# Roywangj/AdaptPoint

Hardware: AMD Instinct MI355X
Metric: set-abstraction fwd+bwd point-clouds/sec (B=32,N=1024) (higher is better)
Workload: dtype bf16

## Files before the change

### adaptpoint_amd/_lib.py

```python
import ctypes
import os

_HERE = os.path.dirname(os.path.abspath(__file__))
LIB_PATH = os.path.join(_HERE, "libadaptpoint_amd.so")
if os.environ.get("APN_LIB_PATH"):
    if os.environ.get("APN_ALLOW_UNSAFE_LIB") != "1":
        raise RuntimeError("APN_LIB_PATH is for diagnostic builds: set APN_ALLOW_UNSAFE_LIB=1 with it")
    LIB_PATH = os.path.abspath(os.environ["APN_LIB_PATH"])
REQUIRED_BUILD_FLAGS = ("-ffp-contract=off", "-fno-slp-vectorize")

_c_int, _c_float, _c_void_p = ctypes.c_int, ctypes.c_float, ctypes.c_void_p
_c_double = ctypes.c_double
_c_longlong = ctypes.c_longlong

SIGNATURES = {
    "apn_version": [],
    "apn_furthest_point_sampling": [_c_int] * 3 + [_c_void_p] * 4,
    "apn_ball_query": [_c_int] * 3 + [_c_float, _c_int] + [_c_void_p] * 4,
    "apn_group_points": [_c_int] * 5 + [_c_void_p] * 4,
    "apn_group_points_grad": [_c_int] * 5 + [_c_void_p] * 4,
    "apn_gather_points": [_c_int] * 4 + [_c_void_p] * 4,
    "apn_gather_points_grad": [_c_int] * 4 + [_c_void_p] * 4,
    "apn_resample_points": [_c_int] * 6 + [_c_void_p] * 6,
    "apn_three_nn": [_c_int] * 3 + [_c_void_p] * 5,
    "apn_three_interpolate": [_c_int] * 4 + [_c_void_p] * 5,
    "apn_three_interpolate_grad": [_c_int] * 4 + [_c_void_p] * 5,
    "apn_furthest_point_sampling_tuned": [_c_int] * 3 + [_c_void_p] * 3 + [_c_int] * 2 + [_c_void_p],
    "apn_fps_debug_stamps": [_c_int] * 3 + [_c_void_p] * 5,
    "apn_furthest_point_sampling_xyz": [_c_int] * 3 + [_c_void_p] * 5,
    "apn_ball_query_zero": [_c_int] * 3 + [_c_float, _c_int] + [_c_void_p] * 4,
    "apn_sa_grid_blocks": [_c_int] * 2,
    "apn_sa_grid_rows": [_c_int] * 3,
    "apn_sa_bwd_main_rows": [_c_int] * 2,
    "apn_sa_acc_words": [_c_int],
    "apn_sa_debug_stamps": [_c_void_p],
    "apn_zero_fill": [_c_void_p, _c_longlong, _c_void_p],
    "apn_debug_stamp": [_c_void_p, _c_int, _c_void_p],
    "apn_debug_vgpr_hold": [_c_int, _c_int, _c_void_p, _c_void_p],
    "apn_debug_vpk_probe": [_c_int, _c_int, _c_int, _c_void_p, _c_void_p],
    "apn_sa_geo_dd_doubles": [_c_int],
    "apn_sa_point_geo": [_c_int] * 4 + [_c_float] + [_c_void_p] * 6,
    "apn_sa_prep_rows": [_c_int] * 2,
    "apn_sa_prep_stats": [_c_int] * 2 + [_c_void_p] * 4 + [_c_int] * 2 + [_c_void_p] * 3 + [_c_longlong, _c_void_p],
    "apn_sa_reduce_rows": [_c_void_p, _c_int, _c_int, _c_double, _c_void_p, _c_void_p],
    "apn_sa_reduce_acc": [_c_void_p, _c_int, _c_double, _c_void_p, _c_void_p],
    "apn_sa_bn_fold": [_c_void_p, _c_int, _c_void_p, _c_int, _c_double, _c_void_p, _c_void_p,
                       _c_float, _c_float, _c_void_p, _c_void_p, _c_void_p, _c_int, _c_void_p,
                       _c_void_p, _c_int, _c_void_p, _c_void_p],
    "apn_sa_fwd_main": [_c_int] * 4 + [_c_float] + [_c_void_p] * 12 + [_c_float, _c_float, _c_int, _c_double,
                                                                        _c_void_p, _c_int] + [_c_void_p] * 7,
    "apn_sa_fwd_out": [_c_int] * 3 + [_c_void_p] * 8 + [_c_float, _c_float, _c_int, _c_double] + [_c_void_p] * 2
                      + [_c_int] + [_c_void_p] * 3 + [_c_int] + [_c_void_p] * 2 + [_c_longlong, _c_void_p],
    "apn_sa_bwd_prep_rows": [_c_int] * 2,
    "apn_sa_bwd_prep": [_c_int] * 3 + [_c_void_p] + [_c_longlong] * 3 + [_c_void_p] + [_c_int]
                       + [_c_void_p] * 3 + [_c_int] + [_c_void_p] * 8,
    "apn_sa_bwd_main": [_c_int] * 4 + [_c_float] + [_c_void_p] * 11 + [_c_double, _c_int] + [_c_void_p] * 9,
    "apn_sa_bwd_weight_rows": [_c_int] * 2,
    "apn_sa_bwd_point_grads": [_c_int] * 3 + [_c_void_p] * 7 + [_c_double, _c_int] + [_c_void_p] * 2 + [_c_int]
                              + [_c_void_p] * 4 + [_c_float] + [_c_void_p] * 5,
    "apn_sa_bwd_finalize": [_c_void_p, _c_int, _c_float, _c_void_p, _c_void_p, _c_int, _c_void_p, _c_void_p, _c_int]
                           + [_c_void_p] * 11,
    "apn_sa_forward_seq": ([_c_int] * 5 + [_c_float] + [_c_void_p] * 12
                           + [_c_void_p] * 5 + [_c_float, _c_float, _c_int]
                           + [_c_void_p] * 5 + [_c_float, _c_float, _c_int]
                           + [_c_double, _c_int] + [_c_void_p] * 11 + [_c_longlong, _c_void_p]),
    "apn_sa_backward_seq": ([_c_int] * 5 + [_c_float] + [_c_void_p] * 15 + [_c_int] * 3
                            + [_c_double] + [_c_void_p] + [_c_longlong] * 3 + [_c_void_p]
                            + [_c_longlong]
                            + [_c_void_p] * 26),
    "apn_attention_small_max": [],
    "apn_attention_small_fwd": [_c_int] * 3 + [_c_void_p] * 5,
    "apn_attention_small_bwd": [_c_int] * 3 + [_c_void_p] * 8,
    "apn_attention_prep": [_c_int] * 3 + [_c_void_p] * 4 + [_c_int, _c_void_p],
    "apn_attention_fwd": [_c_int] * 3 + [_c_void_p] * 4,
    "apn_attention_bwd": [_c_int] * 3 + [_c_void_p] * 9,
    "apn_pointset_group_rows": [_c_int] * 3,
    "apn_pointset_group_max": [_c_int] * 5 + [_c_void_p] * 8,
    "apn_pointset_group_max_grad": [_c_int] * 5 + [_c_void_p] * 9,
    "apn_sa_wide_grid": [_c_int] * 2,
    "apn_sa_wide_colsum_chunks": [_c_int] * 2,
    "apn_sa_wide_colsum": [_c_void_p, _c_int, _c_int, _c_void_p, _c_void_p, _c_void_p],
    "apn_sa_wide_tilemap_ints": [_c_int] * 2,
    "apn_sa_wide_tilemap": [_c_int] * 3 + [_c_void_p] * 3,
    "apn_sa_wide_tilemap_many": [_c_int] * 4 + [_c_void_p] * 3,
    "apn_sa_rowmap_many": [_c_int] * 4 + [_c_void_p] * 6,
    "apn_sa_rowmap_ints": [_c_int] * 2,
    "apn_sa_rowmap_places": [_c_int] * 3,
    "apn_sa_wide_stats1": [_c_int] * 4 + [_c_void_p] * 6,
    "apn_sa_wide_fwd_main": [_c_int] * 5 + [_c_void_p] * 11,
    "apn_sa_wide_bwd_main": [_c_int] * 5 + [_c_void_p] * 15,
    "apn_sa_wide_wgrad_fused": [_c_int],
    "apn_sa_wide_image": [_c_void_p, _c_int, _c_int, _c_void_p, _c_int, _c_int, _c_int, _c_void_p, _c_void_p],
    "apn_sa_wide_bwd_prep_rows": [_c_int] * 2,
    "apn_sa_wide_bwd_prep": [_c_int] * 3 + [_c_void_p] + [_c_longlong] * 3 + [_c_void_p] * 7,
    "apn_sa_wide_consts2": [_c_void_p, _c_int, _c_void_p, _c_int, _c_void_p, _c_double, _c_int] + [_c_void_p] * 4,
    "apn_sa_wide_consts1": [_c_void_p, _c_int, _c_void_p, _c_int, _c_void_p, _c_double, _c_int] + [_c_void_p] * 4,
    "apn_sa_wide_point_terms": [_c_int] * 4 + [_c_void_p] * 5 + [_c_int, _c_float] + [_c_void_p] * 7,
    "apn_sa_wide_wgrad_splits": [_c_int] * 3,
    "apn_sa_wide_csr": [_c_int] * 3 + [_c_void_p] * 9,
    "apn_sa_wide_fwd_prep": [_c_int] * 6 + [_c_float] + [_c_void_p] * 13,
    "apn_sa_wide_fwd_prep_rows": [_c_int] * 3,
    "apn_sa_wide_out": [_c_int] * 3 + [_c_void_p] * 2 + [_c_int] + [_c_void_p] * 3 + [_c_int] + [_c_void_p] * 2,
    "apn_sa_wide_bwd_mid": [_c_void_p, _c_int, _c_void_p, _c_int, _c_int, _c_void_p, _c_double, _c_int] + [_c_void_p] * 7,
    "apn_sa_wide_bwd_fin": [_c_void_p, _c_int, _c_void_p, _c_int, _c_int, _c_void_p, _c_double, _c_int] + [_c_void_p] * 8,
    "apn_sa_wide_point_grads_rows": [_c_int] * 2,
    "apn_sa_wide_point_grads_cols": [_c_int] * 3,
    "apn_sa_wide_point_grads": [_c_int] * 5 + [_c_float] + [_c_void_p] * 13 + [_c_int] + [_c_void_p] * 9,
    "apn_sa_wide_colsum_f32": [_c_void_p, _c_int, _c_int, _c_void_p, _c_void_p],
    "apn_sa_wide_wgrad": [_c_int] * 5 + [_c_void_p] * 7 + [_c_int] + [_c_void_p] * 2,
    "apn_pw_conv_tiles": [_c_int] * 2,
    "apn_pw_conv_forward": [_c_int] * 5 + [_c_void_p] * 5,
    "apn_pw_bn_act": [_c_int] * 3 + [_c_void_p] * 2 + [_c_int] + [_c_void_p] * 2 + [_c_float] * 2 + [_c_int] * 2
                     + [_c_void_p] * 6,
    "apn_pw_bn_act_grad_splits": [_c_int] * 2,
    "apn_pw_bn_act_grad": [_c_int] * 3 + [_c_void_p] * 3 + [_c_int] * 2 + [_c_void_p] * 5,
    "apn_pw_conv_grad_input": [_c_int] * 5 + [_c_void_p] * 4,
    "apn_pw_conv_grad_weight_splits": [_c_int] * 4,
    "apn_pw_conv_grad_weight": [_c_int] * 5 + [_c_void_p] * 5,
    "apn_deform_forward": [_c_int] * 3 + [_c_void_p] * 6 + [_c_float] + [_c_void_p] * 4,
    "apn_deform_backward": [_c_int] * 3 + [_c_void_p] * 4 + [_c_float] + [_c_void_p] * 7,
    "apn_pw_contract_splits": [_c_int] * 4,
    "apn_pw_contract": [_c_int] * 4 + [_c_void_p, _c_longlong, _c_int, _c_int] * 2 + [_c_void_p, _c_longlong, _c_int, _c_int,
                                                                                         _c_void_p, _c_int, _c_void_p],
    "apn_pw_contract2_splits": [_c_int] * 9,
    "apn_pw_contract2": [_c_int] * 3 + [_c_void_p] * 16,
    "apn_fp_blend_stats": [_c_int] * 4 + [_c_void_p] * 6 + [_c_int] + [_c_void_p] * 4 + [_c_float, _c_int] + [_c_void_p] * 3,
    "apn_pw_transpose": [_c_int] * 3 + [_c_void_p] * 3,
    "apn_three_nn_weights": [_c_longlong] + [_c_void_p] * 3,
    "apn_anchor_transforms": [_c_int] + [_c_void_p] * 3 + [_c_float] * 3 + [_c_void_p] * 3,
    "apn_anchor_transforms_grad": [_c_int] + [_c_void_p] * 3 + [_c_float] * 3 + [_c_void_p] * 4,
    "apn_pw_conv_max_tiles": [_c_int],
    "apn_pw_conv_max_forward": [_c_int] * 5 + [_c_void_p] * 3 + [_c_int] + [_c_void_p] * 5,
    "apn_pw_conv_max_backward": [_c_int] * 4 + [_c_void_p] * 5 + [_c_int] + [_c_void_p] * 5,
    "apn_spectral_norm_blocks": [_c_int] * 2,
    "apn_spectral_norm": [_c_int] * 2 + [_c_void_p, _c_int, _c_float] + [_c_void_p] * 8,
    "apn_spectral_norm_grad": [_c_int] * 2 + [_c_void_p] * 8,
    "apn_spectral_norm_many": [_c_int] + [_c_void_p] * 3 + [_c_int, _c_float] + [_c_void_p] * 8,
    "apn_spectral_norm_grad_many": [_c_int] + [_c_void_p] * 10,
    "apn_sa_sample_overlap": [_c_int] * 3 + [_c_float, _c_int] + [_c_void_p] * 7,
    "apn_sa_sample_seq": [_c_int] * 3 + [_c_float, _c_int] + [_c_void_p] * 8,
    "apn_furthest_point_sampling_nested": [_c_int] * 3 + [_c_void_p] * 6,
    "apn_sa_sample_seq_nested": [_c_int] * 3 + [_c_float, _c_int] + [_c_void_p] * 9,
    "apn_pointwolf_params": [_c_int] * 2 + [_c_void_p, _c_int] + [_c_float] * 3 + [_c_void_p] * 4,
    "apn_rsmix_select": [_c_int] * 3 + [_c_void_p] * 2 + [_c_double, _c_int, _c_int] + [_c_void_p] * 3,
    "apn_rsmix_mix": [_c_int] * 4 + [_c_void_p] * 8,
    "apn_cloud_transform": [_c_int] * 4 + [_c_void_p] * 2 + [_c_int] * 2 + [_c_void_p] * 8,
    "apn_cls_confusion": [_c_int] * 2 + [_c_void_p, _c_int] + [_c_void_p] * 5,
    "apn_la_pool_rows": [_c_int] * 2,
    "apn_la_pool_fwd": [_c_int] * 4 + [_c_float] + [_c_void_p] * 3 + [_c_int] + [_c_void_p] * 7,
    "apn_la_stats_fold": [_c_void_p, _c_int, _c_int, _c_double, _c_void_p, _c_void_p],
    "apn_la_pool_bwd": [_c_int] * 4 + [_c_float] + [_c_void_p] * 11 + [_c_int] + [_c_void_p] * 4,
    "apn_knn_query": [_c_int] * 5 + [_c_void_p] * 5,
    "apn_knn_dilated": [_c_int] * 7 + [_c_void_p] * 6,
    "apn_ec_pool_rows": [_c_int] * 2,
    "apn_ec_pool_fwd": [_c_int] * 4 + [_c_void_p, _c_int] + [_c_void_p] * 7,
    "apn_ec_out": [_c_int] * 3 + [_c_void_p] * 2 + [_c_float] + [_c_void_p] * 2,
    "apn_ec_bwd_prep_rows": [_c_int] * 2,
    "apn_ec_bwd_prep": [_c_int] * 3 + [_c_void_p] + [_c_longlong] * 3 + [_c_void_p] * 2 + [_c_float] + [_c_void_p] * 3,
    "apn_ec_out_res": [_c_int] * 3 + [_c_void_p] * 2 + [_c_float, _c_void_p] + [_c_longlong] * 3 + [_c_void_p] * 2,
    "apn_ec_bwd_prep_act": [_c_int] * 3 + [_c_void_p] + [_c_longlong] * 3 + [_c_void_p] * 2 + [_c_float] + [_c_void_p] * 3,
    "apn_ec_csr": [_c_int] * 3 + [_c_void_p] * 5,
    "apn_ec_pool_bwd": [_c_int] * 4 + [_c_void_p] * 5 + [_c_int] + [_c_void_p] * 4,
    "apn_chamfer_max_points": [],
    "apn_chamfer_forward": [_c_int] * 3 + [_c_void_p] * 7,
    "apn_chamfer_backward": [_c_int] * 3 + [_c_void_p] * 9,
    "apn_emd_max_points": [],
    "apn_emd_one_launch_max": [],
    "apn_emd_cost_parts": [_c_int],
    "apn_emd_ratios": [_c_int] * 3 + [_c_void_p] * 6,
    "apn_emd_match": [_c_int] * 3 + [_c_void_p] * 6,
    "apn_emd_cost": [_c_int] * 3 + [_c_void_p] * 8,
    "apn_emd_cost_grad": [_c_int] * 3 + [_c_void_p] * 9,
    "apn_po_knn_query": [_c_int] * 4 + [_c_void_p] * 7,
    "apn_po_ball_query": [_c_int] * 3 + [_c_float, _c_int] + [_c_void_p] * 6,
    "apn_po_furthest_sampling": [_c_int] * 2 + [_c_void_p] * 6,
    "apn_po_csr": [_c_int] * 3 + [_c_void_p] * 5,
    "apn_po_grouping_fwd": [_c_int] * 4 + [_c_void_p] * 4,
    "apn_po_grouping_bwd": [_c_int] * 4 + [_c_void_p] * 5,
    "apn_po_interpolation_fwd": [_c_int] * 4 + [_c_void_p] * 5,
    "apn_po_interpolation_bwd": [_c_int] * 4 + [_c_void_p] * 6,
    "apn_po_subtraction_fwd": [_c_int] * 4 + [_c_void_p] * 5,
    "apn_po_subtraction_bwd": [_c_int] * 4 + [_c_void_p] * 6,
    "apn_po_aggregation_fwd": [_c_int] * 5 + [_c_void_p] * 6,
    "apn_po_aggregation_bwd": [_c_int] * 5 + [_c_void_p] * 11,
    "apn_pt_rows": [_c_int] * 3,
    "apn_pt_mid_rows": [_c_int] * 3,
    "apn_pt_rel_stats": [_c_int] * 3 + [_c_void_p, _c_int] + [_c_void_p] * 5,
    "apn_pt_fold": [_c_void_p, _c_int, _c_int, _c_void_p, _c_void_p],
    "apn_pt_colsum_rows": [_c_int],
    "apn_pt_colsum": [_c_int, _c_int, _c_void_p, _c_int, _c_void_p, _c_void_p],
    "apn_pt_mid": [_c_int] * 3 + [_c_void_p, _c_int] + [_c_void_p] * 7,
    "apn_pt_attend": [_c_int] * 3 + [_c_void_p, _c_int] + [_c_void_p] * 8,
    "apn_pt_attend_bwd": [_c_int] * 3 + [_c_void_p, _c_int] + [_c_void_p] * 10,
    "apn_pt_mid_bwd": [_c_int] * 3 + [_c_void_p, _c_int] + [_c_void_p] * 9,
    "apn_pt_rel_bwd": [_c_int] * 3 + [_c_void_p, _c_int] + [_c_void_p] * 12 + [_c_int, _c_void_p, _c_void_p],
    "apn_pt_scatter_bwd": [_c_int] * 3 + [_c_void_p] * 6 + [_c_int, _c_void_p],
    "apn_vg_scratch_ints": [_c_int],
    "apn_vg_voxelize": [_c_int] * 3 + [_c_void_p] + [_c_double] * 3 + [_c_void_p] * 9,
    "apn_vg_mean_fwd": [_c_int] * 3 + [_c_void_p] * 6,
    "apn_vg_mean_bwd": [_c_int] * 3 + [_c_void_p] * 5,
    "apn_rl_moment_rows": [_c_int] * 3,
    "apn_rl_bwd_rows": [_c_int] * 4,
    "apn_rl_moments": [_c_int] * 3 + [_c_void_p] * 3 + [_c_int] + [_c_void_p] * 3,
    "apn_rl_fold": [_c_int, _c_void_p, _c_double] + [_c_void_p] * 4 + [_c_float, _c_float, _c_int] + [_c_void_p] * 6,
    "apn_rl_forward": [_c_int] * 4 + [_c_void_p] * 3 + [_c_int] + [_c_void_p] * 4,
    "apn_rl_backward": [_c_int] * 4 + [_c_void_p] * 3 + [_c_int] + [_c_void_p] * 6,
    "apn_rl_finalize": [_c_int, _c_int, _c_void_p, _c_void_p, _c_double] + [_c_void_p] * 4 + [_c_int] + [_c_void_p] * 3,
    "apn_ag_moment_rows": [_c_int],
    "apn_ag_point_rows": [_c_int],
    "apn_ag_moments": [_c_int] * 5 + [_c_void_p] * 5,
    "apn_ag_fold": [_c_int] * 2 + [_c_void_p] * 3,
    "apn_ag_combine_fwd": [_c_int] * 5 + [_c_void_p] * 7 + [_c_int] + [_c_void_p] * 4 + [_c_float, _c_int] + [_c_void_p] * 3,
    "apn_ag_combine_bwd": [_c_int] * 5 + [_c_void_p] * 11,
    "apn_ag_sigma_bwd": [_c_int] * 5 + [_c_void_p] * 11,
    "apn_ag_res_relu_max": [_c_int] * 4 + [_c_void_p] * 5,
    "apn_ag_res_relu_max_grad": [_c_int] * 4 + [_c_void_p] * 6,
}

_lib = None


class ExtensionMissing(RuntimeError):
    pass


def load():
    global _lib
    if _lib is not None:
        return _lib
    if not os.path.exists(LIB_PATH):
        raise ExtensionMissing(
            f"{LIB_PATH} not found: build it with `python -m adaptpoint_amd.build` "
            "(hipcc --offload-arch=gfx950). There is no fallback path.")
    lib = ctypes.CDLL(LIB_PATH)
    for name, argtypes in SIGNATURES.items():
        fn = getattr(lib, name)
        fn.argtypes = argtypes
        fn.restype = _c_int
    lib.apn_error_string.argtypes = [_c_int]
    lib.apn_error_string.restype = ctypes.c_char_p
    lib.apn_build_flags.argtypes = []
    lib.apn_build_flags.restype = ctypes.c_char_p
    flags = lib.apn_build_flags().decode("utf-8", "replace").split()
    missing = [f for f in REQUIRED_BUILD_FLAGS if f not in flags]
    if missing and os.environ.get("APN_ALLOW_UNSAFE_LIB") != "1":
        raise ExtensionMissing(f"{LIB_PATH} was built without {missing} (its flags: {' '.join(flags)}): rebuild with "
                               "`python -m adaptpoint_amd.build --force`")
    _lib = lib
    return lib


def check(code, what):
    if code != 0:
        msg = load().apn_error_string(code).decode("utf-8", "replace")
        raise RuntimeError(f"{what} failed: {msg} (code {code})")
```

### adaptpoint_amd/csrc/sa_glue.hip

```cpp
#include "apn_common.h"
#include "sa_chain.h"
#include "apn_mfma.h"

namespace apn {

#ifdef APN_WG_STAMPS
__device__ unsigned long long *d_wg_stamps = nullptr;
__device__ __forceinline__ void wg_stamp(int k) {
    unsigned long long *st = d_wg_stamps;
    if (st && threadIdx.x == 0)
        st[((size_t)blockIdx.y * gridDim.x + blockIdx.x) * 16 + k] = wall_clock64();
}
#else
__device__ __forceinline__ void wg_stamp(int) {}
#endif


typedef __attribute__((ext_vector_type(8))) __bf16 bf16x8;

__device__ __forceinline__ void block_sum_rows(const float *__restrict__ part, int rows, int ncol,
                                               const double *__restrict__ sums, double *out) {
    __shared__ double red[1024 * 4];
    const int t = threadIdx.x;
    if (!part) {
        if (t < ncol) out[t] = sums[t];
        __syncthreads();
        return;
    }
    const int quads = ncol >> 2, q = t % quads, g = t / quads, groups = 1024 / quads;
    const float4 *__restrict__ p4 = (const float4 *)part;
    double s0 = 0.0, s1 = 0.0, s2 = 0.0, s3 = 0.0;
    int r = g;
    for (; r + 7 * groups < rows; r += 8 * groups) {
        float4 v[8];
#pragma unroll
        for (int u = 0; u < 8; ++u) v[u] = p4[(size_t)(r + u * groups) * quads + q];
#pragma unroll
        for (int u = 0; u < 8; ++u) {
            s0 += (double)v[u].x; s1 += (double)v[u].y; s2 += (double)v[u].z; s3 += (double)v[u].w;
        }
    }
    for (; r < rows; r += groups) {
        const float4 v = p4[(size_t)r * quads + q];
        s0 += (double)v.x; s1 += (double)v.y; s2 += (double)v.z; s3 += (double)v.w;
    }
    double *mine = red + (size_t)g * ncol + 4 * q;
    mine[0] = s0; mine[1] = s1; mine[2] = s2; mine[3] = s3;
    __syncthreads();
    for (int st = groups >> 1; st > 0; st >>= 1) {
        if (g < st) {
            const double *other = mine + (size_t)st * ncol;
#pragma unroll
            for (int j = 0; j < 4; ++j) mine[j] += other[j];
        }
        __syncthreads();
    }
    if (t < ncol) out[t] = red[t];
    __syncthreads();
}

__global__ __launch_bounds__(1024) void reduce_rows_kernel(const float *__restrict__ part, int rows,
                                                           int ncol, double count,
                                                           double *__restrict__ out) {
    __shared__ double s[128];
    block_sum_rows(part, rows, ncol, nullptr, s);
    if (threadIdx.x < ncol) out[threadIdx.x] = s[threadIdx.x];
    if (threadIdx.x == 0) { out[ncol] = count; out[ncol + 1] = 1.0; }
}

__device__ __forceinline__ void slice_sum_rows(const float *__restrict__ part, int rows, int quads,
                                               int qa, int qb, double (*red)[4]) {
    const int t = threadIdx.x, grp = t >> 1;
    const float4 *__restrict__ p4 = reinterpret_cast<const float4 *>(part) + ((t & 1) ? qb : qa);
    double s0 = 0.0, s1 = 0.0, s2 = 0.0, s3 = 0.0;
    int r = grp;
    for (; r + 3 * 128 < rows; r += 4 * 128) {
        float4 v[4];
#pragma unroll
        for (int u = 0; u < 4; ++u) v[u] = p4[(size_t)(r + 128 * u) * quads];
#pragma unroll
        for (int u = 0; u < 4; ++u) {
            s0 += (double)v[u].x; s1 += (double)v[u].y; s2 += (double)v[u].z; s3 += (double)v[u].w;
        }
    }
    for (; r < rows; r += 128) {
        const float4 v = p4[(size_t)r * quads];
        s0 += (double)v.x; s1 += (double)v.y; s2 += (double)v.z; s3 += (double)v.w;
    }
    red[t][0] = s0; red[t][1] = s1; red[t][2] = s2; red[t][3] = s3;
    __syncthreads();
    for (int st = 64; st > 0; st >>= 1) {
        if (grp < st) {
#pragma unroll
            for (int j = 0; j < 4; ++j) red[t][j] += red[t + 2 * st][j];
        }
        __syncthreads();
    }
}

__global__ __launch_bounds__(256) void bn_fold_kernel(
    const float *__restrict__ part, int rows, const double *__restrict__ sums_in, int c, double count,
    const float *__restrict__ gamma, const float *__restrict__ beta, float eps, float momentum,
    float *__restrict__ running_mean, float *__restrict__ running_var, long long *__restrict__ nbt,
    int training, float *__restrict__ pack, const float *__restrict__ sgn_gamma, int sgn_c,
    float *__restrict__ sgn_out) {
    __shared__ double red[256][4];
    const int t = threadIdx.x, i = blockIdx.x * 4 + t;
    float g32 = 1.0f, b32 = 0.0f, rm = 0.0f, rv = 1.0f;
    if (t < 4) {
        if (gamma) g32 = gamma[i];
        if (beta) b32 = beta[i];
        if (running_mean) { rm = running_mean[i]; rv = running_var[i]; }
    }
    if (blockIdx.x == 0) {
        if (t == 0 && training && nbt) *nbt += 1;
        if (sgn_out)
            for (int k = t; k < sgn_c; k += 256) sgn_out[k] = (!sgn_gamma || sgn_gamma[k] >= 0.0f) ? 1.0f : -1.0f;
    }
    double sum = 0.0, sumsq = 0.0;
    if (training) {
        if (part) {
            slice_sum_rows(part, rows, c / 2, blockIdx.x, c / 4 + blockIdx.x, red);
            if (t < 4) { sum = red[0][t]; sumsq = red[1][t]; }
        } else if (t < 4) {
            sum = sums_in[i];
            sumsq = sums_in[c + i];
            count = sums_in[2 * c];
        }
    }
    if (t >= 4) return;
    double mean, var;
    if (training) {
        mean = sum / count;
        var = sumsq / count - mean * mean;
        if (var < 0.0) var = 0.0;
        if (running_mean) {
            const double unbiased = var * (count / (count > 1.0 ? count - 1.0 : 1.0));
            running_mean[i] = (float)((1.0 - momentum) * rm + momentum * mean);
            running_var[i] = (float)((1.0 - momentum) * rv + momentum * unbiased);
        }
    } else {
        mean = rm;
        var = rv;
    }
    const double inv = 1.0 / sqrt(var + (double)eps);
    const double g = g32, b = b32;
    pack[i] = (float)(g * inv);
    pack[c + i] = (float)(b - mean * g * inv);
    pack[2 * c + i] = (float)mean;
    pack[3 * c + i] = (float)inv;
}

template <int NT, int QT, int WST, int FST>
__device__ __forceinline__ void stage_skip_operands(int cloud, int n, int m, int m0,
                                                    const __bf16 *__restrict__ ft,
                                                    const __bf16 *__restrict__ ft_lo,
                                                    const int *__restrict__ fidx,
                                                    const float *__restrict__ ws,
                                                    float (*sws)[WST], float (*sfi)[FST], int *ssrc) {
    constexpr int G = NT / 32, QPT = QT / G, WPT = 64 / G;
    const int tid = threadIdx.x, i = tid & 31, q0 = tid >> 5;
    int src[QPT];
#pragma unroll
    for (int t = 0; t < QPT; ++t) {
        const int q = m0 + q0 + G * t;
        const int got = fidx[(size_t)cloud * m + (q < m ? q : m - 1)];
        src[t] = q < m ? got : -1;
    }
    float wv[WPT];
#pragma unroll
    for (int t = 0; t < WPT; ++t) wv[t] = ws[(q0 + G * t) * 32 + i];
    const __bf16 *lo_tab = ft_lo ? ft_lo : ft;
    __bf16 hv[QPT], lv[QPT];
#pragma unroll
    for (int t = 0; t < QPT; ++t) {
        const size_t o = ((size_t)cloud * n + (src[t] < 0 ? 0 : src[t])) * 32 + i;
        hv[t] = ft[o];
        lv[t] = lo_tab[o];
    }
    float v[QPT];
#pragma unroll
    for (int t = 0; t < QPT; ++t) {
        const float f = (float)hv[t] + (ft_lo ? (float)lv[t] : 0.0f);
        v[t] = src[t] >= 0 ? f : 0.0f;
    }
#pragma unroll
    for (int t = 0; t < QPT; ++t) {
        sfi[q0 + G * t][i] = v[t];
        if (ssrc && i == 0) ssrc[q0 + G * t] = src[t] < 0 ? 0 : src[t];
    }
#pragma unroll
    for (int t = 0; t < WPT; ++t) sws[q0 + G * t][i] = wv[t];
}

template <int QT>
__global__ __launch_bounds__(QT * 16) void fwd_out_kernel(int n, int m, const float *__restrict__ ysel,
                                                          const unsigned long long *__restrict__ acc2,
                                                          const double *__restrict__ sums2, BnArgs bn2,
                                                          float *__restrict__ pack2,
                                                          const __bf16 *__restrict__ ft,
                                                          const __bf16 *__restrict__ ft_lo,
                                                          const int *__restrict__ fidx,
                                                          const float *__restrict__ ws,
                                                          const float *__restrict__ bs, int relu,
                                                          float *__restrict__ out, float4 *__restrict__ zero,
                                                          long long zero_n4) {
    constexpr int NT = QT * 16, NW = NT / 64, HALVES = 64 / QT;
    __shared__ float tile[QT][65];
    __shared__ __attribute__((aligned(16))) float sfi[QT][36];
    __shared__ double ftot[128];
    __shared__ float s_sc[64], s_sh[64];
    const bool first = blockIdx.x == 0 && blockIdx.y == 0;
    critical_stream_priority();
    wg_stamp(0);
    double count2 = bn2.count;
    double g2pre = 1.0, b2pre = 0.0;
    if (threadIdx.x < 64) {
        if (bn2.gamma) g2pre = (double)bn2.gamma[threadIdx.x];
        if (bn2.beta) b2pre = (double)bn2.beta[threadIdx.x];
    }
    if (bn2.training) {
        if (threadIdx.x < 128) ftot[threadIdx.x] = sums2 ? sums2[threadIdx.x] : acc_read(acc2, 128, threadIdx.x);
        if (sums2) count2 = sums2[128];
    }
    __shared__ __attribute__((aligned(16))) float sws[64][36];
    __shared__ float s_bs[64];
    const int cloud = blockIdx.y, m0 = blockIdx.x * QT;
    const int tx = threadIdx.x & 63, ty = threadIdx.x >> 6;
    if (threadIdx.x >= 128 && threadIdx.x < 192) s_bs[tx] = (ws && bs) ? bs[tx] : 0.0f;
    float ys4[4];
#pragma unroll
    for (int k = 0; k < 4; ++k) {
        const int q = m0 + ty + NW * k;
        ys4[k] = ysel[((size_t)cloud * m + (q < m ? q : m - 1)) * 64 + tx];
    }
    if (ws) stage_skip_operands<NT, QT, 36, 36>(cloud, n, m, m0, ft, ft_lo, fidx, ws, sws, sfi, nullptr);
    wg_stamp(1);
    __syncthreads();
    wg_stamp(2);
    if (threadIdx.x < 64) {
        if (first && threadIdx.x == 0 && bn2.training && bn2.nbt) *bn2.nbt += 1;
        float sc, sh;
        bn_channel(bn2, 64, threadIdx.x, bn2.training ? ftot[threadIdx.x] : 0.0, bn2.training ? ftot[64 + threadIdx.x] : 0.0,
                   count2, first, pack2, sc, sh, g2pre, b2pre);
        s_sc[threadIdx.x] = sc;
        s_sh[threadIdx.x] = sh;
    }
    __syncthreads();
    {
        const float sc = s_sc[tx], sh = s_sh[tx];
#pragma unroll
        for (int k = 0; k < 4; ++k) {
            const int j = ty + NW * k;
            tile[j][tx] = m0 + j < m ? ys4[k] * sc + sh : 0.f;
        }
    }
    wg_stamp(3);
    __syncthreads();
    wg_stamp(4);
    if (ws) {
        constexpr int QB = QT / 32;
        if (ty < 2 * QB) {
            const int cb = ty & 1, qb = ty >> 1, r = tx & 31, h = tx >> 5;
            f32x16 acc = {0};
#pragma unroll
            for (int st = 0; st < 2; ++st) {
                float av[8], bv[8];
                const float4 a0 = *reinterpret_cast<const float4 *>(&sws[32 * cb + r][16 * st + 8 * h]);
                const float4 a1 = *reinterpret_cast<const float4 *>(&sws[32 * cb + r][16 * st + 8 * h + 4]);
                const float4 b0 = *reinterpret_cast<const float4 *>(&sfi[32 * qb + r][16 * st + 8 * h]);
                const float4 b1 = *reinterpret_cast<const float4 *>(&sfi[32 * qb + r][16 * st + 8 * h + 4]);
                av[0] = a0.x; av[1] = a0.y; av[2] = a0.z; av[3] = a0.w; av[4] = a1.x; av[5] = a1.y; av[6] = a1.z; av[7] = a1.w;
                bv[0] = b0.x; bv[1] = b0.y; bv[2] = b0.z; bv[3] = b0.w; bv[4] = b1.x; bv[5] = b1.y; bv[6] = b1.z; bv[7] = b1.w;
                acc = mfma<2>(make_frag<2>(av), make_frag<2>(bv), acc);
            }
            const int ql = 32 * qb + r;
#pragma unroll
            for (int e = 0; e < 16; ++e) {
                const int c = 32 * cb + acc_row(e, h);
                float v = tile[ql][c] + (acc[e] + s_bs[c]);
                if (relu) v = fmaxf(v, 0.0f);
                if (m0 + ql < m) out[((size_t)cloud * 64 + c) * m + m0 + ql] = v;
            }
        }
    } else {
        const int ql = tx % QT, hh = tx / QT;
#pragma unroll
        for (int k = 0; k < 4; ++k) {
            const int c = 4 * (ty * HALVES + hh) + k;
            float v = tile[ql][c];
            if (relu) v = fmaxf(v, 0.0f);
            if (m0 + ql < m) out[((size_t)cloud * 64 + c) * m + m0 + ql] = v;
        }
    }
    wg_stamp(5);
    if (zero) {
        const long long nb = (long long)gridDim.x * gridDim.y, bid = (long long)blockIdx.y * gridDim.x + blockIdx.x;
        for (long long i = bid * NT + threadIdx.x; i < zero_n4; i += nb * NT) zero[i] = make_float4(0.f, 0.f, 0.f, 0.f);
    }
    wg_stamp(6);
}

template <int QT>
__global__ __launch_bounds__(QT * 16) void bwd_prep_kernel(int n, int m, const float *__restrict__ g_out,
                                                           long long gs_b, long long gs_c, long long gs_m,
                                                           const float *__restrict__ out, int relu,
                                                           const float *__restrict__ ysel,
                                                           const float *__restrict__ pack2,
                                                           const __bf16 *__restrict__ ft,
                                                           const __bf16 *__restrict__ ft_lo,
                                                           const int *__restrict__ fidx,
                                                           const float *__restrict__ ws,
                                                           float *__restrict__ goa,
                                                           unsigned long long *__restrict__ accS,
                                                           float *__restrict__ partWs,
                                                           float *__restrict__ gip,
                                                           const int *__restrict__ dup) {
    constexpr int NT = QT * 16, NW = NT / 64, HALVES = 64 / QT;
    __shared__ float tile[QT][65];
    __shared__ float red[NW][2][64];
    __shared__ __attribute__((aligned(16))) float sfi[QT][36];
    __shared__ float sws[64][33];
    __shared__ int ssrc[QT];
    constexpr int DW = QT == 32 ? 4 : 2;
    __shared__ float sdfi[DW][QT][33];
    const int cloud = blockIdx.y, m0 = blockIdx.x * QT;
    const int tx = threadIdx.x & 63, ty = threadIdx.x >> 6;
    const int ql = tx % QT, hh = tx / QT;
    critical_stream_priority();
    wg_stamp(0);
    const bool distinct = dup && dup[cloud] == 0;
    const int qc = m0 + ql < m ? m0 + ql : m - 1;
    const float *outp = relu ? out : g_out;
    float gv[4], ov[4];
#pragma unroll
    for (int k = 0; k < 4; ++k) {
        const int c = (ty + NW * k) * HALVES + hh;
        gv[k] = g_out[cloud * gs_b + c * gs_c + qc * gs_m];
        ov[k] = relu ? outp[((size_t)cloud * 64 + c) * m + qc] : 1.0f;
    }
    float ys[4];
#pragma unroll
    for (int k = 0; k < 4; ++k) {
        const int q = m0 + ty + NW * k;
        ys[k] = ysel[((size_t)cloud * m + (q < m ? q : m - 1)) * 64 + tx];
    }
    if (ws) stage_skip_operands<NT, QT, 33, 36>(cloud, n, m, m0, ft, ft_lo, fidx, ws, sws, sfi, ssrc);
#pragma unroll
    for (int k = 0; k < 4; ++k) {
        const int c = (ty + NW * k) * HALVES + hh;
        tile[ql][c] = (m0 + ql < m && ov[k] > 0.0f) ? gv[k] : 0.0f;
    }
    const float sc = pack2[tx], mu = pack2[128 + tx], iv = pack2[192 + tx];
    wg_stamp(1);
    __syncthreads();
    wg_stamp(2);
    float s1 = 0.0f, s2 = 0.0f;
#pragma unroll
    for (int k = 0; k < 4; ++k) {
        const int j = ty + NW * k, q = m0 + j;
        if (q < m) {
            const float g = tile[j][tx];
            const float gs = g * sc;
            goa[((size_t)cloud * m + q) * 64 + tx] = gs;
            s1 += g;
            s2 += g * ((ys[k] - mu) * iv);
        }
    }
    red[ty][0][tx] = s1;
    red[ty][1][tx] = s2;
    wg_stamp(3);
    __syncthreads();
    wg_stamp(4);
    const size_t blk = (size_t)blockIdx.y * gridDim.x + blockIdx.x;
    float sacc = 0.0f;
    if (ty < 2) {
#pragma unroll
        for (int k = 0; k < NW; ++k) sacc += red[k][ty][tx];
    }
    wg_stamp(5);
    if (ws) {
        constexpr int QB = QT / 32;
        const int r = tx & 31, h = tx >> 5;
        if (ty < DW * QB) {
            const int qb = ty / DW, part = ty % DW;
            f32x16 acc = {0};
#pragma unroll
            for (int s4 = 0; s4 < 4 / DW; ++s4) {
                const int st = (4 / DW) * part + s4;
                float av[8], bv[8];
#pragma unroll
                for (int j = 0; j < 8; ++j) {
                    av[j] = tile[32 * qb + r][16 * st + 8 * h + j];
                    bv[j] = sws[16 * st + 8 * h + j][r];
                }
                acc = mfma<2>(make_frag<2>(av), make_frag<2>(bv), acc);
            }
#pragma unroll
            for (int e = 0; e < 16; ++e)
                sdfi[part][32 * qb + acc_row(e, h)][r] = acc[e];
        } else if (ty < DW * QB + 2) {
            const int cb = ty - DW * QB;
            f32x16 acc = {0};
#pragma unroll
            for (int st = 0; st < QT / 16; ++st) {
                float av[8], bv[8];
#pragma unroll
                for (int j = 0; j < 8; ++j) {
                    av[j] = tile[16 * st + 8 * h + j][32 * cb + r];
                    bv[j] = sfi[16 * st + 8 * h + j][r];
                }
                acc = mfma<2>(make_frag<2>(av), make_frag<2>(bv), acc);
            }
#pragma unroll
            for (int e = 0; e < 16; ++e)
                partWs[blk * 2048 + (32 * cb + acc_row(e, h)) * 32 + r] = acc[e];
        }
        __syncthreads();
#pragma unroll
        for (int k = 0; k < QT * 32 / NT; ++k) {
            const int o = threadIdx.x + NT * k, q = o >> 5, i = o & 31;
            float v = sdfi[0][q][i] + sdfi[1][q][i];
            if (DW == 4) v += sdfi[DW - 2][q][i] + sdfi[DW - 1][q][i];
            float *dst = gip + ((size_t)cloud * n + ssrc[q]) * 32 + i;
            if (m0 + q < m) {
                if (distinct) *dst = v;
                else atomicAdd(dst, v);
            }
        }
        wg_stamp(6);
    }
    if (ty < 2) acc_add(accS, 128, (int)(blk % ACC_COPIES), ty * 64 + tx, sacc);
    wg_stamp(7);
}

constexpr int WG_PTS = 64;
constexpr int PG_NT = 512, PG_K = WG_PTS * 32 / PG_NT, PG_M = 32 * 64 / PG_NT;
constexpr int PG_RB = 8;

__global__ __launch_bounds__(PG_NT) void bwd_point_grads_kernel(
    int n, int total_q, int split, const float *__restrict__ GU, const int *__restrict__ pcnt,
    const int *__restrict__ poff, const long long *__restrict__ geo,
    const float *__restrict__ HA, const float *__restrict__ HB, const unsigned long long *__restrict__ accT,
    const double *__restrict__ sumsT, double count, int train1,
    const float *__restrict__ pack1, const __bf16 *__restrict__ ft,
    const __bf16 *__restrict__ ft_lo, const float *__restrict__ xyz,
    const float *__restrict__ new_xyz, const float *__restrict__ w1, const float *__restrict__ gip,
    float inv_r, float *__restrict__ partW, float *__restrict__ g_f, float *__restrict__ g_p,
    float *__restrict__ g_q) {
    __shared__ __attribute__((aligned(16))) float swt[35][36];
    __shared__ __attribute__((aligned(16))) float swr[32][36];
    __shared__ float sG[WG_PTS][33];
    __shared__ float sH[WG_PTS][33];
    __shared__ float sI[WG_PTS][33];
    __shared__ float sB[WG_PTS][41];
    __shared__ float sGeo[WG_PTS][4];
    __shared__ float sc[5][32];
    const int tid = threadIdx.x;
    critical_stream_priority();
    wg_stamp(0);
    const int cloud = blockIdx.y, n0 = blockIdx.x * WG_PTS;
    const int block = cloud * gridDim.x + blockIdx.x;
    const size_t p0 = (size_t)cloud * n + n0;
    const int q0 = block * WG_PTS;
    const int n_here = n - n0 < WG_PTS ? n - n0 : WG_PTS;
    const int c_ld = tid & 31;
    float f_hi[PG_K], f_lo[PG_K], g_i[PG_K], h_a[PG_K], h_b[PG_K];
    const int g_pt = tid >> 3, g_c4 = (tid & 7) * 4;
    int r_cnt, r_off;
    {
        const size_t gp = p0 + (g_pt < n_here ? g_pt : 0);
        r_cnt = g_pt < n_here ? pcnt[gp] : 0;
        r_off = poff[gp];
    }
    float4 a_g = make_float4(0.f, 0.f, 0.f, 0.f);
    {
        const __bf16 *lo_tab = ft_lo ? ft_lo : ft;
        const float *gip_tab = gip ? gip : HA;
#pragma unroll
        for (int k = 0; k < PG_K; ++k) {
            const int pt = (tid >> 5) + (PG_NT / 32) * k;
            const size_t pr = (p0 + (pt < n_here ? pt : 0)) * 32 + c_ld;
            const size_t qr = (size_t)(q0 + pt < total_q ? q0 + pt : 0) * 32 + c_ld;
            f_hi[k] = (float)ft[pr];
            f_lo[k] = (float)lo_tab[pr];
            g_i[k] = gip_tab[gip ? pr : qr];
            h_a[k] = HA[qr];
            h_b[k] = HB[qr];
        }
    }
    float xq_v[2] = {0.0f, 0.0f};
    long long geo_v = 0ll;
    if (tid < WG_PTS * 3) {
        const int pt = tid / 3, d = tid % 3;
        xq_v[0] = xyz[(p0 + (pt < n_here ? pt : 0)) * 3 + d];
        xq_v[1] = new_xyz[(size_t)(q0 + pt < total_q ? q0 + pt : 0) * 3 + d];
    } else if (tid >= PG_NT - WG_PTS * 4) {
        const int e = tid - (PG_NT - WG_PTS * 4), pt = e >> 2, j = e & 3;
        geo_v = geo[(p0 + (pt < n_here ? pt : 0)) * 4 + j];
    }
    for (int e = tid; e < 32 * 35; e += PG_NT) {
        const int mid = e / 35, col = e % 35;
        const float w = w1[e];
        const __bf16 hi = (__bf16)w;
        float wr = (float)hi;
        if (split) wr += (float)(__bf16)(w - wr);
        swt[col][mid] = w;
        swr[mid][col < 3 ? 32 + col : col - 3] = wr;
    }
    if (tid < 64) {
        const int c = tid & 31;
        const float sca = pack1[c];
        float val = 0.0f;
        if (train1) {
            const double t = sumsT ? sumsT[tid] : acc_read(accT, 64, tid);
            const double cnt = sumsT ? sumsT[64] : count;
            val = (float)(-(double)sca * t / cnt);
        }
        sc[tid < 32 ? 2 : 1][c] = val;
        if (tid < 32) sc[0][c] = sca;
    } else if (tid >= 96 && tid < 160) sc[3 + ((tid - 96) >> 5)][tid & 31] = pack1[64 + tid - 96];
    {
        const float *rows = GU + (size_t)(r_cnt > 0 ? r_off : 0) * 32 + g_c4;
        for (int j0 = 0; j0 < r_cnt; j0 += PG_RB) {
            float4 v[PG_RB];
#pragma unroll
            for (int u = 0; u < PG_RB; ++u) {
                const int j = j0 + u < r_cnt ? j0 + u : r_cnt - 1;
                v[u] = *reinterpret_cast<const float4 *>(rows + (size_t)j * 32);
            }
#pragma unroll
            for (int u = 0; u < PG_RB; ++u)
                if (j0 + u < r_cnt) { a_g.x += v[u].x; a_g.y += v[u].y; a_g.z += v[u].z; a_g.w += v[u].w; }
        }
    }
    wg_stamp(1);
    __syncthreads();
    wg_stamp(2);
    {
        const int c = tid & 31;
        const float ca = sc[0][c], cb = sc[1][c], cc = sc[2][c];
#pragma unroll
        for (int k = 0; k < PG_K; ++k) {
            const int pt = (tid >> 5) + (PG_NT / 32) * k;
            const bool ok = pt < n_here;
            sB[pt][6 + c] = ok ? f_hi[k] + (ft_lo ? f_lo[k] : 0.0f) : 0.0f;
            sI[pt][c] = (gip && ok) ? g_i[k] : 0.0f;
            sH[pt][c] = q0 + pt < total_q ? __builtin_fmaf(ca, h_a[k], __builtin_fmaf(cb, h_b[k], cc * 32.0f)) : 0.0f;
        }
    }
    sG[g_pt][g_c4] = a_g.x; sG[g_pt][g_c4 + 1] = a_g.y;
    sG[g_pt][g_c4 + 2] = a_g.z; sG[g_pt][g_c4 + 3] = a_g.w;
    if (tid < WG_PTS * 3) {
        const int pt = tid / 3, d = tid % 3;
        const float xv = xq_v[0], qv = xq_v[1];
        sB[pt][d] = pt < n_here ? xv : 0.0f;
        sB[pt][3 + d] = q0 + pt < total_q ? qv : 0.0f;
        sB[pt][38 + d] = 0.0f;
    } else if (tid >= PG_NT - WG_PTS * 4) {
        const int e = tid - (PG_NT - WG_PTS * 4), pt = e >> 2, j = e & 3;
        const long long gv = pt < n_here ? geo_v : 0ll;
        sGeo[pt][j] = j == 0 ? (float)gv : (float)((double)gv * (1.0 / 68719476736.0));
    }
    wg_stamp(3);
    __syncthreads();
    wg_stamp(4);

    const int tx = tid & 63, ty = tid >> 6;
    {
        const float cnt = sGeo[tx][0], gx = sGeo[tx][1], gy = sGeo[tx][2], gz = sGeo[tx][3];
        float fx[32];
#pragma unroll
        for (int i = 0; i < 32; ++i) fx[i] = sB[tx][6 + i];
#pragma unroll
        for (int mm = 0; mm < PG_M; ++mm) {
            const int mid = PG_M * ty + mm;
            const float4 *wrow = reinterpret_cast<const float4 *>(swr[mid]);
            float accf = 0.0f;
#pragma unroll
            for (int i4 = 0; i4 < 8; ++i4) {
                const float4 w = wrow[i4];
                accf = __builtin_fmaf(w.x, fx[4 * i4], accf);
                accf = __builtin_fmaf(w.y, fx[4 * i4 + 1], accf);
                accf = __builtin_fmaf(w.z, fx[4 * i4 + 2], accf);
                accf = __builtin_fmaf(w.w, fx[4 * i4 + 3], accf);
            }
            const float4 wx = wrow[8];
            const float ys = wx.x * gx + wx.y * gy + wx.z * gz + cnt * accf;
            const float yhs = sc[4][mid] * (ys - cnt * sc[3][mid]);
            sG[tx][mid] = sc[0][mid] * sG[tx][mid] + sc[1][mid] * yhs + sc[2][mid] * cnt;
        }
    }
    wg_stamp(5);
    __syncthreads();
    wg_stamp(6);

    {
        const int r = tx & 31, h = tx >> 5;
        if (ty < 3) {
            const float (*X)[33] = ty == 2 ? sH : sG;
            const int col = ty == 1 ? 32 + r : r;
            const bool mine = ty == 0 ? !(r >= 3 && r <= 5) : (ty == 1 ? r < 6 : (r >= 3 && r <= 5));
            f32x16 acc = {0};
#pragma unroll
            for (int st = 0; st < WG_PTS / 16; ++st) {
                float av[8], bv[8];
#pragma unroll
                for (int j = 0; j < 8; ++j) {
                    av[j] = X[16 * st + 8 * h + j][r];
                    bv[j] = mine ? sB[16 * st + 8 * h + j][col] : 0.0f;
                }
                acc = mfma<2>(make_frag<2>(av), make_frag<2>(bv), acc);
            }
            float *row = partW + (size_t)block * 32 * 38;
            if (mine) {
#pragma unroll
                for (int e = 0; e < 16; ++e) row[acc_row(e, h) * 38 + col] = acc[e];
            }
        } else if (ty < 5) {
            const int pb = ty - 3;
            f32x16 acc = {0};
#pragma unroll
            for (int st = 0; st < 2; ++st) {
                float av[8], bv[8];
                const float4 a0 = *reinterpret_cast<const float4 *>(&swt[3 + r][16 * st + 8 * h]);
                const float4 a1 = *reinterpret_cast<const float4 *>(&swt[3 + r][16 * st + 8 * h + 4]);
                av[0] = a0.x; av[1] = a0.y; av[2] = a0.z; av[3] = a0.w; av[4] = a1.x; av[5] = a1.y; av[6] = a1.z; av[7] = a1.w;
#pragma unroll
                for (int j = 0; j < 8; ++j) bv[j] = sG[32 * pb + r][16 * st + 8 * h + j];
                acc = mfma<2>(make_frag<2>(av), make_frag<2>(bv), acc);
            }
            const int pt = 32 * pb + r;
#pragma unroll
            for (int e = 0; e < 16; ++e) {
                const int i = acc_row(e, h);
                if (pt < n_here) g_f[((size_t)cloud * 32 + i) * n + n0 + pt] = acc[e] + sI[pt][i];
            }
        }
    }
    if (!g_p && !g_q) {
        wg_stamp(7);
        return;
    }

    float gr[32];
#pragma unroll
    for (int mid = 0; mid < 32; ++mid) gr[mid] = sG[tx][mid];
    auto dot_col = [&](const float (&v)[32], int col) {
        const float4 *wcol = reinterpret_cast<const float4 *>(swt[col]);
        float s = 0.0f;
#pragma unroll
        for (int i4 = 0; i4 < 8; ++i4) {
            const float4 w = wcol[i4];
            s = __builtin_fmaf(v[4 * i4], w.x, s);
            s = __builtin_fmaf(v[4 * i4 + 1], w.y, s);
            s = __builtin_fmaf(v[4 * i4 + 2], w.z, s);
            s = __builtin_fmaf(v[4 * i4 + 3], w.w, s);
        }
        return s;
    };
    if (ty < 3 && g_p && tx < n_here) g_p[(p0 + tx) * 3 + ty] += dot_col(gr, ty) * inv_r;
    if (ty >= 4 && ty < 7 && g_q && q0 + tx < total_q) {
        float hr[32];
#pragma unroll
        for (int mid = 0; mid < 32; ++mid) hr[mid] = sH[tx][mid];
        g_q[(size_t)(q0 + tx) * 3 + ty - 4] = -dot_col(hr, ty - 4) * inv_r;
    }
    wg_stamp(7);
}

constexpr int FIN_COLS = 32, FIN_GROUPS = 16;
__device__ __forceinline__ double col_sum(const float *__restrict__ base, int rows, int stride,
                                          int col, int g) {
    double s = 0.0;
    int r = g;
    for (; r + 15 * FIN_GROUPS < rows; r += 16 * FIN_GROUPS) {
        float v[16];
#pragma unroll
        for (int u = 0; u < 16; ++u) v[u] = base[(size_t)(r + FIN_GROUPS * u) * stride + col];
#pragma unroll
        for (int u = 0; u < 16; ++u) s += (double)v[u];
    }
    for (; r + 3 * FIN_GROUPS < rows; r += 4 * FIN_GROUPS) {
        float v[4];
#pragma unroll
        for (int u = 0; u < 4; ++u) v[u] = base[(size_t)(r + FIN_GROUPS * u) * stride + col];
#pragma unroll
        for (int u = 0; u < 4; ++u) s += (double)v[u];
    }
    for (; r < rows; r += FIN_GROUPS) s += (double)base[(size_t)r * stride + col];
    return s;
}

constexpr int FIN_W1 = 32 * 35, FIN_WS = 2048, FIN_W2 = 2048, FIN_SMALL = 64 * 3 + 32 * 2;
constexpr int FIN_TOTAL = FIN_W1 + FIN_WS + FIN_W2 + FIN_SMALL;

__global__ __launch_bounds__(FIN_COLS * FIN_GROUPS) void bwd_finalize_kernel(
    const float *__restrict__ partW, int rowsW, double inv_r, float *__restrict__ g_w1,
    const float *__restrict__ partWs, int rowsS, float *__restrict__ g_ws,
    const float *__restrict__ partW2, int rows2, float *__restrict__ g_w2,
    const unsigned long long *__restrict__ accS, const double *__restrict__ sumsS,
    const unsigned long long *__restrict__ accT, const double *__restrict__ sumsT,
    float *__restrict__ g_bs, float *__restrict__ g_g2, float *__restrict__ g_b2, float *__restrict__ g_g1,
    float *__restrict__ g_b1) {
    __shared__ double red[FIN_GROUPS][FIN_COLS];
    critical_stream_priority();
    const int o = threadIdx.x % FIN_COLS, g = threadIdx.x / FIN_COLS;
    const int e = blockIdx.x * FIN_COLS + o;
    double v = 0.0;
    float *dst = nullptr;
    if (e < FIN_W1) {
        const int mid = e / 35, col = e % 35;
        dst = g_w1 + e;
        if (col < 3)
            v = (col_sum(partW, rowsW, 1216, mid * 38 + col, g) -
                 col_sum(partW, rowsW, 1216, mid * 38 + 3 + col, g)) * inv_r;
        else
            v = col_sum(partW, rowsW, 1216, mid * 38 + 3 + col, g);
    } else if (e < FIN_W1 + FIN_WS) {
        if (g_ws) { dst = g_ws + (e - FIN_W1); v = col_sum(partWs, rowsS, 2048, e - FIN_W1, g); }
    } else if (e < FIN_W1 + FIN_WS + FIN_W2) {
        if (g_w2) { dst = g_w2 + (e - FIN_W1 - FIN_WS); v = col_sum(partW2, rows2, 2048, e - FIN_W1 - FIN_WS, g); }
    } else if (e < FIN_TOTAL) {
        if (g == 0) {
            const int k = e - FIN_W1 - FIN_WS - FIN_W2;
            if (k < 192) {
                const int c = k & 63, which = k >> 6;
                const double scale = (sumsS && which) ? 1.0 / sumsS[129] : 1.0;
                if (which == 0) {
                    if (g_bs) { dst = g_bs + c; v = acc_read(accS, 128, c); }
                } else {
                    const int col = which == 1 ? c : 64 + c;
                    dst = which == 1 ? (g_b2 ? g_b2 + c : nullptr) : (g_g2 ? g_g2 + c : nullptr);
                    if (dst) v = (sumsS ? sumsS[col] : acc_read(accS, 128, col)) * scale;
                }
            } else {
                const int c = (k - 192) & 31, which = (k - 192) >> 5;
                const double scale = sumsT ? 1.0 / sumsT[65] : 1.0;
                dst = which == 0 ? (g_b1 ? g_b1 + c : nullptr) : (g_g1 ? g_g1 + c : nullptr);
                if (dst) v = (sumsT ? sumsT[32 * which + c] : acc_read(accT, 64, 32 * which + c)) * scale;
            }
        }
    }
    red[g][o] = v;
    __syncthreads();
    if (g == 0 && dst) {
        double acc = 0.0;
#pragma unroll
        for (int k = 0; k < FIN_GROUPS; ++k) acc += red[k][o];
        *dst = (float)acc;
    }
}

__global__ __launch_bounds__(128) void reduce_acc_kernel(const unsigned long long *__restrict__ acc, int ncol,
                                                         double count, double *__restrict__ out) {
    const int t = threadIdx.x;
    if (t < ncol) out[t] = acc_read(acc, ncol, t);
    if (t == 0) { out[ncol] = count; out[ncol + 1] = 1.0; }
}

}

#define APN_ST ((hipStream_t)stream)

extern "C" int apn_sa_reduce_rows(const float *part, int rows, int ncol, double count, double *out,
                                  void *stream) {
    if (rows < 0 || ncol < 4 || ncol > 128 || (1024 % ncol) || !part || !out) return APN_EINVAL;
    if ((uintptr_t)part & 15) return APN_EINVAL;
    hipLaunchKernelGGL(apn::reduce_rows_kernel, dim3(1), dim3(1024), 0, APN_ST, part, rows, ncol, count,
                       out);
    APN_LAUNCH_CHECK();
    return APN_OK;
}

extern "C" int apn_sa_reduce_acc(const void *acc, int ncol, double count, double *out, void *stream) {
    if (ncol < 1 || ncol > 128 || !acc || !out) return APN_EINVAL;
    hipLaunchKernelGGL(apn::reduce_acc_kernel, dim3(1), dim3(128), 0, APN_ST, (const unsigned long long *)acc, ncol,
                       count, out);
    APN_LAUNCH_CHECK();
    return APN_OK;
}

extern "C" int apn_sa_bn_fold(const float *part, int rows, const double *sums, int c, double count,
                              const float *gamma, const float *beta, float eps, float momentum,
                              float *running_mean, float *running_var, void *num_batches_tracked,
                              int training, float *pack, const float *sgn_gamma, int sgn_c,
                              float *sgn_out, void *stream) {
    if (c < 4 || c > 1024 || (c & 3) || !pack || sgn_c > 1024) return APN_EINVAL;
    if (training && !part && !sums) return APN_EINVAL;
    if (!training && (!running_mean || !running_var)) return APN_EINVAL;
    if (part && ((uintptr_t)part & 15)) return APN_EINVAL;
    hipLaunchKernelGGL(apn::bn_fold_kernel, dim3(c / 4), dim3(256), 0, APN_ST, part, rows, sums, c, count,
                       gamma, beta, eps, momentum, running_mean, running_var,
                       (long long *)num_batches_tracked, training, pack, sgn_gamma, sgn_c, sgn_out);
    APN_LAUNCH_CHECK();
    return APN_OK;
}

static int apn_sa_glue_tile(int b, int m) { return (long long)b * ((m + 63) / 64) <= 512 ? 32 : 64; }

extern "C" int apn_sa_fwd_out(int b, int n, int m, const float *ysel, const void *acc2, const double *sums2,
                              const float *g2, const float *b2, float *rm2, float *rv2, void *nbt2, float eps2,
                              float mom2, int train2, double count, float *pack2, const void *ft, int precision,
                              const int *fidx, const float *ws, const float *bs, int relu, float *out,
                              float *zero_base, long long zero_floats, void *stream) {
    if (b <= 0 || m <= 0 || b > 65535 || !ysel || !pack2 || !out) return APN_EINVAL;
    if (train2 && !acc2 && !sums2) return APN_EINVAL;
    if (!train2 && (!rm2 || !rv2)) return APN_EINVAL;
    if (ws && (!ft || !fidx || n <= 0 || (precision != 1 && precision != 2))) return APN_EINVAL;
    const __bf16 *hi = (const __bf16 *)ft;
    const __bf16 *lo = (ws && precision == 2) ? hi + (size_t)b * n * 32 : nullptr;
    if (zero_base && (zero_floats < 0 || (zero_floats & 3) || ((uintptr_t)zero_base & 15))) return APN_EINVAL;
    apn::BnArgs bn{g2, b2, rm2, rv2, (long long *)nbt2, eps2, mom2, train2, count};
    if (apn_sa_glue_tile(b, m) == 32)
        hipLaunchKernelGGL(apn::fwd_out_kernel<32>, dim3((m + 31) / 32, b), dim3(512), 0, APN_ST, n, m, ysel,
                           (const unsigned long long *)(sums2 ? nullptr : acc2), sums2, bn, pack2, hi, lo, fidx, ws, bs,
                           relu, out, (float4 *)zero_base, zero_base ? zero_floats / 4 : 0);
    else
        hipLaunchKernelGGL(apn::fwd_out_kernel<64>, dim3((m + 63) / 64, b), dim3(1024), 0, APN_ST, n, m, ysel,
                           (const unsigned long long *)(sums2 ? nullptr : acc2), sums2, bn, pack2, hi, lo, fidx, ws, bs,
                           relu, out, (float4 *)zero_base, zero_base ? zero_floats / 4 : 0);
    APN_LAUNCH_CHECK();
    return APN_OK;
}

extern "C" int apn_sa_bwd_prep_rows(int b, int m) {
    const int qt = apn_sa_glue_tile(b, m);
    return b * ((m + qt - 1) / qt);
}

extern "C" int apn_sa_bwd_prep(int b, int n, int m, const float *g_out, long long gs_b,
                               long long gs_c, long long gs_m, const float *out, int relu,
                               const float *ysel, const float *pack2, const void *ft, int precision,
                               const int *fidx, const float *ws, float *goa, void *accS,
                               float *partWs, float *gip, const int *dup, void *stream) {
    if (b <= 0 || m <= 0 || b > 65535 || !g_out || !ysel || !pack2 || !goa || !accS) return APN_EINVAL;
    if (relu && !out) return APN_EINVAL;
    if (ws && (!ft || !fidx || !partWs || !gip || n <= 0 || (precision != 1 && precision != 2)))
        return APN_EINVAL;
    const __bf16 *hi = (const __bf16 *)ft;
    const __bf16 *lo = (ws && precision == 2) ? hi + (size_t)b * n * 32 : nullptr;
    if (apn_sa_glue_tile(b, m) == 32)
        hipLaunchKernelGGL(apn::bwd_prep_kernel<32>, dim3((m + 31) / 32, b), dim3(512), 0, APN_ST, n, m, g_out,
                           gs_b, gs_c, gs_m, out, relu, ysel, pack2, hi, lo, fidx, ws, goa, (unsigned long long *)accS,
                           partWs, gip, dup);
    else
        hipLaunchKernelGGL(apn::bwd_prep_kernel<64>, dim3((m + 63) / 64, b), dim3(1024), 0, APN_ST, n, m, g_out,
                           gs_b, gs_c, gs_m, out, relu, ysel, pack2, hi, lo, fidx, ws, goa, (unsigned long long *)accS,
                           partWs, gip, dup);
    APN_LAUNCH_CHECK();
    return APN_OK;
}

#ifdef APN_WG_STAMPS
extern "C" __attribute__((visibility("default"))) int apn_sa_debug_wg_stamps(void *buf) {
    return (int)hipMemcpyToSymbol(HIP_SYMBOL(apn::d_wg_stamps), &buf, sizeof(buf));
}
#endif

extern "C" int apn_sa_bwd_weight_rows(int b, int n) { return b * ((n + apn::WG_PTS - 1) / apn::WG_PTS); }

extern "C" int apn_sa_bwd_point_grads(int b, int n, int m, const float *GU, const int *pcnt_poff, const void *geo,
                                      const float *HA, const float *HB, const void *accT, const double *sumsT,
                                      double count, int train1, const float *pack1, const void *ft, int precision,
                                      const float *xyz, const float *new_xyz, const float *w1,
                                      const float *gip, float radius, float *partW, float *g_f,
                                      float *g_p, float *g_newp, void *stream) {
    if (b <= 0 || n <= 0 || m <= 0 || b > 65535) return APN_EINVAL;
    if (!GU || !pcnt_poff || !geo || !HA || !HB || (!accT && !sumsT) || !pack1 || !ft || !xyz || !new_xyz || !w1 || !partW ||
        !g_f)
        return APN_EINVAL;
    if (precision != 1 && precision != 2) return APN_EINVAL;
    if (m > n) return APN_EINVAL;
    const __bf16 *hi = (const __bf16 *)ft;
    const __bf16 *lo = precision == 2 ? hi + (size_t)b * n * 32 : nullptr;
    hipLaunchKernelGGL(apn::bwd_point_grads_kernel, dim3((n + apn::WG_PTS - 1) / apn::WG_PTS, b),
                       dim3(apn::PG_NT), 0, APN_ST, n, b * m, precision == 2 ? 1 : 0, GU, pcnt_poff,
                       pcnt_poff + (size_t)b * n, (const long long *)geo, HA, HB,
                       (const unsigned long long *)accT, sumsT, count, train1,
                       pack1, hi, lo, xyz, new_xyz, w1, gip, 1.0f / radius, partW, g_f, g_p, g_newp);
    APN_LAUNCH_CHECK();
    return APN_OK;
}

extern "C" int apn_sa_bwd_finalize(const float *partW, int rows_w, float radius, float *g_w1,
                                   const float *partWs, int rows_s, float *g_ws, const float *partW2, int rows_2,
                                   float *g_w2, const void *accS, const double *sumsS,
                                   const void *accT, const double *sumsT, float *g_bs, float *g_g2, float *g_b2,
                                   float *g_g1, float *g_b1, void *stream) {
    if (!partW || !g_w1 || (g_ws && !partWs) || (g_w2 && !partW2) || !accS || (!accT && !sumsT))
        return APN_EINVAL;
    hipLaunchKernelGGL(apn::bwd_finalize_kernel, dim3((apn::FIN_TOTAL + apn::FIN_COLS - 1) / apn::FIN_COLS),
                       dim3(apn::FIN_COLS * apn::FIN_GROUPS), 0, APN_ST, partW,
                       rows_w, 1.0 / (double)radius, g_w1, partWs, rows_s, g_ws, partW2, rows_2, g_w2,
                       (const unsigned long long *)accS, sumsS, (const unsigned long long *)accT, sumsT, g_bs,
                       g_g2, g_b2, g_g1, g_b1);
    APN_LAUNCH_CHECK();
    return APN_OK;
}
```

### adaptpoint_amd/csrc/sa_seq.hip

```cpp
#include "apn_common.h"

#define APN_TRY(expr)            \
    do {                         \
        int rc__ = (expr);       \
        if (rc__) return rc__;   \
    } while (0)

namespace apn {
__global__ __launch_bounds__(256) void zero16_kernel(uint4 *__restrict__ p, long long n16) {
    const long long stride = (long long)gridDim.x * 256;
    for (long long e = (long long)blockIdx.x * 256 + threadIdx.x; e < n16; e += stride) p[e] = make_uint4(0, 0, 0, 0);
}
__global__ __launch_bounds__(256) void fill32_kernel(unsigned *__restrict__ p, unsigned word, long long n) {
    const long long stride = (long long)gridDim.x * 256;
    for (long long e = (long long)blockIdx.x * 256 + threadIdx.x; e < n; e += stride) p[e] = word;
}
}

extern "C" int apn_zero_fill(void *base, long long bytes, void *stream) {
    if (bytes < 0 || (bytes & 15) || (bytes && (!base || ((uintptr_t)base & 15)))) return APN_EINVAL;
    if (!bytes) return APN_OK;
    long long blocks = (bytes / 16 + 255) / 256;
    if (blocks > 1024) blocks = 1024;
    hipLaunchKernelGGL(apn::zero16_kernel, dim3((unsigned)blocks), dim3(256), 0, (hipStream_t)stream, (uint4 *)base,
                       bytes / 16);
    APN_LAUNCH_CHECK();
    return APN_OK;
}

extern "C" int apn_sa_forward_seq(
    int phases, int precision, int b, int n, int m, float radius, const float *xyz, const float *new_xyz,
    const float *f, const int *idx, const int *tmap, const int *fidx, const void *geo, const void *dd,
    const float *w1, const float *w2, const float *ws, const float *bs,
    const float *g1, const float *b1, float *rm1, float *rv1, void *nbt1, float eps1, float mom1,
    int train1,
    const float *g2, const float *b2, float *rm2, float *rv2, void *nbt2, float eps2, float mom2,
    int train2,
    double count, int relu, void *ft, float *part1, const double *sums1, const double *sums2,
    float *pack1, float *pack2, void *acc2, float *ysel, void *ksel,
    float *out, float *zero_base, long long zero_floats, void *stream) {
    if (phases & 1)
        APN_TRY(apn_sa_prep_stats(b, n, f, geo, dd, w1, precision, train1, ft, part1, acc2, apn_sa_acc_words(128),
                                  stream));
    if (phases & 2)
        APN_TRY(apn_sa_fwd_main(b, n, m, precision, radius, xyz, new_xyz, ft, idx, tmap, w1, w2, g1, b1, rm1, rv1,
                                nbt1, eps1, mom1, train1, count, part1, apn_sa_prep_rows(b, n), sums1, pack1, g2,
                                ysel, ksel, acc2, stream));
    if (phases & 4)
        APN_TRY(apn_sa_fwd_out(b, n, m, ysel, acc2, sums2, g2, b2, rm2, rv2, nbt2, eps2, mom2, train2, count, pack2,
                               ws ? ft : nullptr, precision, ws ? fidx : nullptr, ws, bs, relu, out, zero_base,
                               zero_floats, stream));
    return APN_OK;
}

extern "C" int apn_sa_backward_seq(
    int phases, int precision, int b, int n, int m, float radius, const float *xyz, const float *new_xyz,
    const int *idx, const int *tmap, const int *fidx, const void *geo, const float *w1, const float *w2,
    const float *ws, const void *ft, const float *pack1, const float *pack2, const float *ysel,
    const void *ksel, const float *out, int relu, int train1, int train2, double count,
    const float *g_out, long long gs_b, long long gs_c, long long gs_m,
    void *zero_base, long long zero_bytes, float *gip, void *accS, void *accT,
    const int *pcnt_poff, const int *rowdst, float *GU,
    float *goa, float *partWs, float *partW2, float *partW, const double *sumsS, const double *sumsT,
    float *HA, float *HB,
    float *g_f, float *g_p, float *g_newp, float *g_w1, float *g_w2, float *g_g1, float *g_b1, float *g_g2,
    float *g_b2, float *g_ws, float *g_bs, void *stream) {
    if (phases & 1) {
        if (zero_bytes) APN_TRY(apn_zero_fill(zero_base, zero_bytes, stream));
        APN_TRY(apn_sa_bwd_prep(b, n, m, g_out, gs_b, gs_c, gs_m, out, relu, ysel, pack2, ws ? ft : nullptr, precision,
                                ws ? fidx : nullptr, ws, goa, accS, partWs, gip,
                                pcnt_poff ? pcnt_poff + 2ll * b * n : nullptr, stream));
    }
    if (phases & 2)
        APN_TRY(apn_sa_bwd_main(b, n, m, precision, radius, xyz, new_xyz, ft, idx, tmap, w1, w2, pack1, pack2, accS,
                                sumsS, count, train2, goa, ksel, accT, partW2, rowdst, GU, HA, HB, stream));
    if (phases & 4) {
        APN_TRY(apn_sa_bwd_point_grads(b, n, m, GU, pcnt_poff, geo, HA, HB, accT, sumsT, count, train1, pack1, ft, precision, xyz,
                                       new_xyz, w1, gip, radius, partW, g_f, g_p, g_newp, stream));
        APN_TRY(apn_sa_bwd_finalize(partW, apn_sa_bwd_weight_rows(b, n), radius, g_w1, partWs,
                                    apn_sa_bwd_prep_rows(b, m), g_ws, partW2, apn_sa_bwd_main_rows(b, m), g_w2, accS,
                                    sumsS, accT, sumsT, g_bs, g_g2, g_b2, g_g1, g_b1, stream));
    }
    return APN_OK;
}

extern "C" int apn_sa_sample_seq_nested(int b, int n, int m, float radius, int nsample, const float *xyz,
                                        const int *tie_prev, int *tie_out, int *fidx, float *new_xyz, int *idx, void *geo,
                                        void *dd, void *stream) {
    if (b <= 0 || n <= 0 || m <= 0 || !tie_out) return APN_EINVAL;
    APN_TRY(apn_furthest_point_sampling_nested(b, n, m, xyz, tie_prev, fidx, new_xyz, tie_out, stream));
    APN_TRY(apn_ball_query_zero(b, n, m, radius, nsample, new_xyz, xyz, idx, stream));
    if (geo) APN_TRY(apn_sa_point_geo(b, n, m, nsample, radius, xyz, new_xyz, idx, geo, dd, stream));
    return APN_OK;
}

extern "C" int apn_sa_sample_seq(int b, int n, int m, float radius, int nsample, const float *xyz,
                                 float *temp, int *fidx, float *new_xyz, int *idx, void *geo, void *dd,
                                 void *stream) {
    if (b <= 0 || n <= 0 || m <= 0) return APN_EINVAL;
    if (temp) {
        long long blocks = ((long long)b * n + 255) / 256;
        if (blocks > 2048) blocks = 2048;
        hipLaunchKernelGGL(apn::fill32_kernel, dim3((unsigned)blocks), dim3(256), 0, (hipStream_t)stream, (unsigned *)temp,
                           0x501502F9u, (long long)b * n);
        APN_LAUNCH_CHECK();
    }
    APN_TRY(apn_furthest_point_sampling_xyz(b, n, m, xyz, temp, fidx, new_xyz, stream));
    APN_TRY(apn_ball_query_zero(b, n, m, radius, nsample, new_xyz, xyz, idx, stream));
    if (geo) APN_TRY(apn_sa_point_geo(b, n, m, nsample, radius, xyz, new_xyz, idx, geo, dd, stream));
    return APN_OK;
}
```

### adaptpoint_amd/fused.py

```python
import torch
import torch.distributed as dist
import torch.nn as nn

from . import _lib
from . import ops as _ops

C_IN, C_MID, C_OUT, K_NS = 32, 32, 64, 32
DETERMINISTIC = True

PRECISION = "bf16x3"
_PREC = {"bf16": 1, "bf16x3": 2}

PER_KERNEL_LAUNCH = False


def covers(B, N, M, K, C, w1, w2, biased=False, momenta=()):
    return (C == C_IN and K == K_NS and tuple(w1) == (C_MID, C_IN + 3) and tuple(w2) == (C_OUT, C_MID) and not biased
            and (M is None or M <= N) and B <= 65535 and all(m is not None for m in momenta))


def supported(p, f, idx_or_k, conv1, conv2, bns=(), npoint=None):
    k = idx_or_k.shape[2] if torch.is_tensor(idx_or_k) else int(idx_or_k)
    m = idx_or_k.shape[1] if torch.is_tensor(idx_or_k) else npoint
    return (f.is_cuda and f.dtype == torch.float32 and p.dtype == torch.float32
            and covers(p.shape[0], p.shape[1], m, k, f.shape[1], conv1.weight.shape[:2], conv2.weight.shape[:2],
                       conv1.bias is not None or conv2.bias is not None, [bn.momentum for bn in bns]))


_FN = {}


def _call(name, dev, *args, stream=None):
    fn = _FN.get(name)
    if fn is None:
        fn = _FN[name] = getattr(_lib.load(), name)
    if stream is None:
        if dev.index is not None and dev.index != torch.cuda.current_device():
            with torch.cuda.device(dev):
                code = fn(*args, torch.cuda.current_stream(dev).cuda_stream)
            if code:
                _lib.check(code, name)
            return
        stream = torch.cuda.current_stream(dev).cuda_stream
    code = fn(*args, stream)
    if code:
        _lib.check(code, name)


class _Launcher:

    def __init__(self, dev):
        self.dev = dev
        if dev.index is not None and dev.index != torch.cuda.current_device():
            self.stream = None
        else:
            self.stream = torch.cuda.current_stream(dev).cuda_stream

    def __call__(self, name, *args):
        _call(name, self.dev, *args, stream=self.stream)


def _ptr(t):
    return None if t is None else t.data_ptr()


FORCE_PHASED = False


def _world(sync):
    if sync and dist.is_available() and dist.is_initialized():
        return dist.get_world_size()
    return 1


def _allreduce_sum_(t):
    if dist.is_available() and dist.is_initialized() and (dist.get_world_size() > 1 or FORCE_PHASED):
        from . import dp
        dp.all_reduce_sum_(t)


def _phased(sync):
    return _world(sync) > 1 or (FORCE_PHASED and sync)


def _carve(dev, sizes, zero=False):
    offs, total = [], 0
    for _, nfl in sizes:
        offs.append(total)
        total += (int(nfl) + 63) // 64 * 64
    buf = (torch.zeros if zero else torch.empty)(max(total, 64), dtype=torch.float32, device=dev)
    return {name: buf[o:o + int(nfl)] for (name, nfl), o in zip(sizes, offs)}, buf


def _all_reduce_rows(call, part, rows, ncol, count, dev):
    sums = torch.empty(ncol + 2, dtype=torch.float64, device=dev)
    call("apn_sa_reduce_rows", part.data_ptr(), rows, ncol, float(count), sums.data_ptr())
    _allreduce_sum_(sums)
    return sums


def _all_reduce_acc(call, acc, ncol, count, dev):
    sums = torch.empty(ncol + 2, dtype=torch.float64, device=dev)
    call("apn_sa_reduce_acc", acc.data_ptr(), ncol, float(count), sums.data_ptr())
    _allreduce_sum_(sums)
    return sums


def _bn_args(bn):
    training = bn.training or not bn.track_running_stats
    track = bn.track_running_stats
    if bn.momentum is None:
        raise RuntimeError("fused set abstraction: BatchNorm(momentum=None) is not covered "
                           "(fused.supported() routes it to the unfused path)")
    mom = bn.momentum
    return (_ptr(bn.weight), _ptr(bn.bias), _ptr(bn.running_mean) if track else None,
            _ptr(bn.running_var) if track else None,
            _ptr(bn.num_batches_tracked) if (track and bn.training) else None,
            float(bn.eps), float(mom), 1 if training else 0)


def _mat(w, rows, cols):
    w = w.detach().reshape(rows, cols)
    return w if w.is_contiguous() else w.contiguous()


def _acc_floats(ncol):
    return 2 * _lib.load().apn_sa_acc_words(ncol)


class _Forward:

    def __init__(self, p, f, new_p, idx, fidx, radius, conv1, bn1, conv2, bn2, skip_conv, relu,
                 sync_bn, tmap=None, geo=None, dd=None, want_backward=False, rowmap=None):
        dev = f.device
        call = _Launcher(dev)
        lib = _lib.load()
        B, C, N = f.shape
        M = new_p.shape[1]
        self.dims = (B, N, M)
        self.radius = float(radius)
        self.sync = sync_bn
        self.relu = 1 if relu else 0
        self.prec = prec = _PREC[PRECISION]
        w1 = _mat(conv1.weight, C_MID, C_IN + 3)
        w2 = _mat(conv2.weight, C_OUT, C_MID)
        ws = bs = None
        if skip_conv is not None:
            ws = _mat(skip_conv.weight, C_OUT, C_IN)
            bs = skip_conv.bias.detach() if skip_conv.bias is not None else None
        count = float(B * M * K_NS)
        if geo is None:
            geo, dd = point_geo(p, new_p, idx, radius)
        if want_backward:
            from . import fused_wide
            if tmap is None:
                tmap = fused_wide.tile_map(idx)
                rowmap = None
            if rowmap is None:
                rowmap = fused_wide.row_map(tmap, B, N, M, fidx=fidx)
        rows1 = lib.apn_sa_prep_rows(B, N)
        v, _buf = _carve(dev, [("ft", prec * B * N * C // 2), ("pack1", 4 * C_MID), ("pack2", 4 * C_OUT),
                               ("ysel", B * M * C_OUT), ("ksel", B * M * C_OUT // 4),
                               ("part1", rows1 * 64), ("acc2", _acc_floats(128))])
        out = torch.empty(B, C_OUT, M, dtype=torch.float32, device=dev)
        self.zsizes = (([("gip", B * N * C_MID)] if ws is not None else [])
                       + [("accS", _acc_floats(128)), ("accT", _acc_floats(64))])
        self.zviews = self.zbuf = None
        if want_backward:
            self.zviews, self.zbuf = _carve(dev, self.zsizes)
        zptr, zfl = _ptr(self.zbuf), (self.zbuf.numel() if self.zbuf is not None else 0)
        bn1a, bn2a = _bn_args(bn1), _bn_args(bn2)
        self.train1, self.train2 = bool(bn1a[7]), bool(bn2a[7])

        def run(phases, sums1=None, sums2=None):
            if PER_KERNEL_LAUNCH:
                return _forward_per_kernel(call, phases, prec, B, N, M, self.radius, p, new_p, f, idx, fidx, geo, dd,
                                           w1, w2, ws, bs, bn1a, bn2a, count, self.relu, v, sums1,
                                           sums2, out, rows1, tmap, zptr, zfl)
            call("apn_sa_forward_seq", phases, prec, B, N, M, self.radius, p.data_ptr(), new_p.data_ptr(),
                 f.data_ptr(), idx.data_ptr(), _ptr(tmap), _ptr(fidx), geo.data_ptr(), dd.data_ptr(),
                 w1.data_ptr(), w2.data_ptr(), _ptr(ws), _ptr(bs), *bn1a, *bn2a, count, self.relu,
                 v["ft"].data_ptr(), v["part1"].data_ptr(), _ptr(sums1), _ptr(sums2),
                 v["pack1"].data_ptr(), v["pack2"].data_ptr(), v["acc2"].data_ptr(),
                 v["ysel"].data_ptr(), v["ksel"].data_ptr(), out.data_ptr(), zptr, zfl)

        if not _phased(sync_bn):
            run(7)
        else:
            run(1)
            s1 = _all_reduce_rows(call, v["part1"], rows1, 64, count, dev) if self.train1 else None
            run(2, sums1=s1)
            s2 = _all_reduce_acc(call, v["acc2"], 128, count, dev) if self.train2 else None
            run(4, sums2=s2)
        self.out = out
        self.saved = dict(p=p, f=f, new_p=new_p, idx=idx, tmap=tmap, rowmap=rowmap, fidx=fidx,
                          geo=geo, ft=v["ft"], w1=w1, w2=w2, ws=ws,
                          has_bs=bs is not None, pack1=v["pack1"], pack2=v["pack2"], ysel=v["ysel"],
                          ksel=v["ksel"], count=count)


def _backward(fw, g_out, need_p, need_newp):
    if fw is None:
        raise RuntimeError("fused set abstraction: backward called a second time (its saved state is "
                           "released after the first backward; retain_graph is not supported)")
    sv = fw.saved
    B, N, M = fw.dims
    dev = fw.out.device
    P, sync = sv["count"], fw.sync
    f32 = dict(dtype=torch.float32, device=dev)
    if g_out is None:
        g_out = torch.zeros_like(fw.out)
    if g_out.dtype != torch.float32:
        g_out = g_out.float()
    gs = g_out.stride()
    w1, w2, ws = sv["w1"], sv["w2"], sv["ws"]
    has_skip = ws is not None
    lib = _lib.load()
    call = _Launcher(dev)
    rows = lib.apn_sa_bwd_main_rows(B, M)
    prow = lib.apn_sa_bwd_prep_rows(B, M)
    wrows = lib.apn_sa_bwd_weight_rows(B, N)

    prezeroed = fw.zbuf is not None
    zsizes = [] if prezeroed else fw.zsizes
    if sv["rowmap"] is None:
        raise RuntimeError("fused set abstraction: backward without a row map (the forward was run with want_backward=False)")
    pcnt_poff, rowdst = sv["rowmap"]
    sizes = zsizes + [("goa", B * M * C_OUT), ("partWs", prow * C_OUT * C_IN if has_skip else 0),
                      ("partW2", rows * C_OUT * C_MID), ("partW", wrows * 32 * 38),
                      ("HA", B * M * C_MID), ("HB", B * M * C_MID), ("GU", lib.apn_sa_rowmap_places(B, N, M) * C_MID)]
    v, buf = _carve(dev, sizes)
    zero_floats = sum((nfl + 63) // 64 * 64 for _, nfl in zsizes)
    if prezeroed:
        v.update(fw.zviews)
        fw.zbuf = fw.zviews = None
    gsz = [("w2", C_OUT * C_MID), ("w1", C_MID * (C_IN + 3)), ("g1", C_MID), ("b1", C_MID),
           ("g2", C_OUT), ("b2", C_OUT), ("ws", C_OUT * C_IN if has_skip else 0),
           ("bs", C_OUT if (has_skip and sv["has_bs"]) else 0)]
    g, _gbuf = _carve(dev, gsz)
    g_f = torch.empty(B, C_IN, N, **f32)
    g_p = _ops.zeros(B, N, 3, **f32) if need_p else None
    g_newp = torch.empty(B, M, 3, **f32) if need_newp else None
    gws = g["ws"].data_ptr() if has_skip else None
    gbs = g["bs"].data_ptr() if (has_skip and sv["has_bs"]) else None

    def run(phases, sumsS=None, sumsT=None):
        if PER_KERNEL_LAUNCH:
            return _backward_per_kernel(call, phases, fw, sv, g_out, buf, zero_floats, v, g, sumsS,
                                        sumsT, g_f, g_p, g_newp, rows, prow, wrows, has_skip, pcnt_poff, rowdst)
        call("apn_sa_backward_seq", phases, fw.prec, B, N, M, fw.radius, sv["p"].data_ptr(),
             sv["new_p"].data_ptr(), sv["idx"].data_ptr(), _ptr(sv["tmap"]), _ptr(sv["fidx"]), sv["geo"].data_ptr(),
             w1.data_ptr(), w2.data_ptr(), _ptr(ws), sv["ft"].data_ptr(), sv["pack1"].data_ptr(),
             sv["pack2"].data_ptr(), sv["ysel"].data_ptr(), sv["ksel"].data_ptr(),
             fw.out.data_ptr(), fw.relu, 1 if fw.train1 else 0, 1 if fw.train2 else 0, float(P),
             g_out.data_ptr(), gs[0], gs[1], gs[2], buf.data_ptr(), zero_floats * 4,
             v["gip"].data_ptr() if has_skip else None, v["accS"].data_ptr(),
             v["accT"].data_ptr(), pcnt_poff.data_ptr(), rowdst.data_ptr(), v["GU"].data_ptr(), v["goa"].data_ptr(),
             v["partWs"].data_ptr() if has_skip else None, v["partW2"].data_ptr(), v["partW"].data_ptr(),
             _ptr(sumsS), _ptr(sumsT), v["HA"].data_ptr(), v["HB"].data_ptr(),
             g_f.data_ptr(), _ptr(g_p), _ptr(g_newp), g["w1"].data_ptr(), g["w2"].data_ptr(),
             g["g1"].data_ptr(), g["b1"].data_ptr(), g["g2"].data_ptr(), g["b2"].data_ptr(), gws, gbs)

    if not _phased(sync):
        run(7)
    else:
        run(1)
        sS = _all_reduce_acc(call, v["accS"], 128, P, dev)
        run(2, sumsS=sS)
        sT = _all_reduce_acc(call, v["accT"], 64, P, dev)
        run(4, sumsS=sS, sumsT=sT)
    return dict(f=g_f, p=g_p, new_p=g_newp, w1=g["w1"].view(C_MID, C_IN + 3, 1, 1),
                w2=g["w2"].view(C_OUT, C_MID, 1, 1), g1=g["g1"], b1=g["b1"], g2=g["g2"], b2=g["b2"],
                ws=g["ws"].view(C_OUT, C_IN, 1) if has_skip else None,
                bs=g["bs"] if (has_skip and sv["has_bs"]) else None)


def _forward_per_kernel(call, phases, prec, B, N, M, radius, p, new_p, f, idx, fidx, geo, dd, w1, w2, ws, bs,
                        bn1a, bn2a, count, relu, v, sums1, sums2, out, rows1, tmap=None, zptr=None, zfl=0):
    lib = _lib.load()
    if phases & 1:
        call("apn_sa_prep_stats", B, N, f.data_ptr(), geo.data_ptr(), dd.data_ptr(), w1.data_ptr(), prec,
             bn1a[7], v["ft"].data_ptr(), v["part1"].data_ptr(), v["acc2"].data_ptr(), lib.apn_sa_acc_words(128))
    if phases & 2:
        call("apn_sa_fwd_main", B, N, M, prec, radius, p.data_ptr(), new_p.data_ptr(), v["ft"].data_ptr(),
             idx.data_ptr(), _ptr(tmap), w1.data_ptr(), w2.data_ptr(), *bn1a, count, v["part1"].data_ptr(), rows1,
             _ptr(sums1), v["pack1"].data_ptr(), bn2a[0], v["ysel"].data_ptr(), v["ksel"].data_ptr(),
             v["acc2"].data_ptr())
    if phases & 4:
        call("apn_sa_fwd_out", B, N, M, v["ysel"].data_ptr(), v["acc2"].data_ptr(), _ptr(sums2), *bn2a, count,
             v["pack2"].data_ptr(), v["ft"].data_ptr() if ws is not None else None, prec,
             _ptr(fidx) if ws is not None else None, _ptr(ws), _ptr(bs), relu, out.data_ptr(), zptr, zfl)


def _backward_per_kernel(call, phases, fw, sv, g_out, buf, zero_floats, v, g, sumsS, sumsT, g_f, g_p,
                         g_newp, rows, prow, wrows, has_skip, pcnt_poff, rowdst):
    B, N, M = fw.dims
    w1, w2, ws, P = sv["w1"], sv["w2"], sv["ws"], float(sv["count"])
    gip = v["gip"].data_ptr() if has_skip else None
    if phases & 1:
        if zero_floats:
            call("apn_zero_fill", buf.data_ptr(), zero_floats * 4)
        call("apn_sa_bwd_prep", B, N, M, g_out.data_ptr(), *g_out.stride(), fw.out.data_ptr(), fw.relu,
             sv["ysel"].data_ptr(), sv["pack2"].data_ptr(), sv["ft"].data_ptr() if has_skip else None,
             fw.prec, _ptr(sv["fidx"]) if has_skip else None, _ptr(ws), v["goa"].data_ptr(),
             v["accS"].data_ptr(), v["partWs"].data_ptr() if has_skip else None, gip,
             pcnt_poff.data_ptr() + 8 * B * N)
    if phases & 2:
        call("apn_sa_bwd_main", B, N, M, fw.prec, fw.radius, sv["p"].data_ptr(), sv["new_p"].data_ptr(),
             sv["ft"].data_ptr(), sv["idx"].data_ptr(), _ptr(sv["tmap"]), w1.data_ptr(), w2.data_ptr(),
             sv["pack1"].data_ptr(), sv["pack2"].data_ptr(), v["accS"].data_ptr(), _ptr(sumsS), P,
             1 if fw.train2 else 0, v["goa"].data_ptr(), sv["ksel"].data_ptr(), v["accT"].data_ptr(),
             v["partW2"].data_ptr(), rowdst.data_ptr(), v["GU"].data_ptr(), v["HA"].data_ptr(), v["HB"].data_ptr())
    if phases & 4:
        call("apn_sa_bwd_point_grads", B, N, M, v["GU"].data_ptr(), pcnt_poff.data_ptr(), sv["geo"].data_ptr(),
             v["HA"].data_ptr(), v["HB"].data_ptr(), v["accT"].data_ptr(), _ptr(sumsT), P, 1 if fw.train1 else 0,
             sv["pack1"].data_ptr(), sv["ft"].data_ptr(), fw.prec, sv["p"].data_ptr(), sv["new_p"].data_ptr(),
             w1.data_ptr(), gip, fw.radius, v["partW"].data_ptr(), g_f.data_ptr(), _ptr(g_p), _ptr(g_newp))
        call("apn_sa_bwd_finalize", v["partW"].data_ptr(), wrows, fw.radius, g["w1"].data_ptr(),
             v["partWs"].data_ptr() if has_skip else None, prow, g["ws"].data_ptr() if has_skip else None,
             v["partW2"].data_ptr(), rows, g["w2"].data_ptr(), v["accS"].data_ptr(), _ptr(sumsS),
             v["accT"].data_ptr(), _ptr(sumsT), g["bs"].data_ptr() if (has_skip and sv["has_bs"]) else None,
             g["g2"].data_ptr(), g["b2"].data_ptr(), g["g1"].data_ptr(), g["b1"].data_ptr())


class _GroupedMlpMax(torch.autograd.Function):
    @staticmethod
    def forward(ctx, p, new_p, f, idx, w1, g1, b1, w2, g2, b2, mods):
        radius, conv1, bn1, conv2, bn2, sync_bn = mods
        fw = _Forward(p.contiguous(), f.contiguous(), new_p.contiguous(), idx.contiguous(), None,
                      radius, conv1, bn1, conv2, bn2, None, False, sync_bn, want_backward=any(ctx.needs_input_grad))
        ctx.fw = fw
        ctx.save_for_backward(p, new_p, f, idx)
        ctx.set_materialize_grads(False)
        ctx.flags = (p.requires_grad, new_p.requires_grad,
                     g1 is not None, b1 is not None, g2 is not None, b2 is not None)
        return fw.out

    @staticmethod
    def backward(ctx, g_out):
        need_p, need_q, a1, a2, a3, a4 = ctx.flags
        ctx.saved_tensors
        g = _backward(ctx.fw, g_out, need_p, need_q)
        ctx.fw = None
        return (g["p"], g["new_p"], g["f"], None, g["w1"], g["g1"] if a1 else None,
                g["b1"] if a2 else None, g["w2"], g["g2"] if a3 else None,
                g["b2"] if a4 else None, None)


def grouped_mlp_max(p, new_p, f, idx, radius, conv1, bn1, conv2, bn2, sync_bn=False):
    return _GroupedMlpMax.apply(p, new_p, f, idx, conv1.weight, bn1.weight, bn1.bias,
                                conv2.weight, bn2.weight, bn2.bias,
                                (radius, conv1, bn1, conv2, bn2, sync_bn))


class Sampling:

    def __init__(self, B, M, K, device):
        self.shape = (B, M, K)
        self.buf = torch.empty(B * M * (1 + 3 + K), dtype=torch.int32, device=device)
        o = 0
        self.fidx = self.buf[o:o + B * M].view(B, M)
        o += B * M
        self.new_p = self.buf[o:o + B * M * 3].view(torch.float32).view(B, M, 3)
        o += B * M * 3
        self.idx = self.buf[o:o + B * M * K].view(B, M, K)
        self.index = None
        self.tmap = None
        self.rowmap = None
        self.geo = None
        self.dd = None
        self.ready = None
        self.ties = None

    def alloc_geo(self, n_points):
        if self.geo is None or self.geo.shape[1] != n_points:
            B = self.shape[0]
            dev = self.buf.device
            self.geo = torch.empty(B, n_points, 4, dtype=torch.int64, device=dev)
            self.dd = torch.empty(B, _lib.load().apn_sa_geo_dd_doubles(n_points), dtype=torch.float64, device=dev)
        return self.geo, self.dd

    def clouds(self, lo, hi):
        v = object.__new__(Sampling)
        for name, t in vars(self).items():
            setattr(v, name, t[lo:hi] if name in _PER_CLOUD and t is not None else None)
        v.shape = (hi - lo,) + self.shape[1:]
        return v


_PER_CLOUD = ("fidx", "new_p", "idx", "geo", "dd", "ties")


@torch.no_grad()
def point_geo(p, new_p, idx, radius, out=None):
    B, N, _ = p.shape
    M, K = idx.shape[1], idx.shape[2]
    dev = p.device
    if out is None:
        geo = torch.empty(B, N, 4, dtype=torch.int64, device=dev)
        dd = torch.empty(B, _lib.load().apn_sa_geo_dd_doubles(N), dtype=torch.float64, device=dev)
    else:
        geo, dd = out
    _Launcher(dev)("apn_sa_point_geo", B, N, M, K, float(radius), p.contiguous().data_ptr(),
                   new_p.contiguous().data_ptr(), idx.contiguous().data_ptr(), geo.data_ptr(), dd.data_ptr())
    return geo, dd


@torch.no_grad()
def sample_and_query(p, npoint, radius, nsample=K_NS, out=None, geo=False, nested=False, ties=None):
    p = p.contiguous()
    dev = p.device
    B, N, _ = p.shape
    smp = out if out is not None else Sampling(B, npoint, nsample, dev)
    assert smp.shape == (B, npoint, nsample)
    gptr = dptr = None
    if geo and nsample == K_NS and smp.buf is not None:
        g_, d_ = smp.alloc_geo(N)
        gptr, dptr = g_.data_ptr(), d_.data_ptr()
    elif geo and nsample == K_NS and smp.geo is not None:
        gptr, dptr = smp.geo.data_ptr(), smp.dd.data_ptr()
    call = _Launcher(dev)
    if nested and N <= 4096:
        if smp.ties is None:
            smp.ties = torch.empty(B, dtype=torch.int32, device=dev)
        if PER_KERNEL_LAUNCH:
            call("apn_furthest_point_sampling_nested", B, N, npoint, p.data_ptr(), _ptr(ties), smp.fidx.data_ptr(),
                 smp.new_p.data_ptr(), smp.ties.data_ptr())
            call("apn_ball_query_zero", B, N, npoint, float(radius), nsample, smp.new_p.data_ptr(), p.data_ptr(),
                 smp.idx.data_ptr())
            if gptr is not None:
                call("apn_sa_point_geo", B, N, npoint, nsample, float(radius), p.data_ptr(), smp.new_p.data_ptr(),
                     smp.idx.data_ptr(), gptr, dptr)
            return smp
        call("apn_sa_sample_seq_nested", B, N, npoint, float(radius), nsample, p.data_ptr(), _ptr(ties), smp.ties.data_ptr(),
             smp.fidx.data_ptr(), smp.new_p.data_ptr(), smp.idx.data_ptr(), gptr, dptr)
        return smp
    if PER_KERNEL_LAUNCH:
        call("apn_furthest_point_sampling_xyz", B, N, npoint, p.data_ptr(), None,
             smp.fidx.data_ptr(), smp.new_p.data_ptr())
        call("apn_ball_query_zero", B, N, npoint, float(radius), nsample, smp.new_p.data_ptr(),
             p.data_ptr(), smp.idx.data_ptr())
        if gptr is not None:
            call("apn_sa_point_geo", B, N, npoint, nsample, float(radius), p.data_ptr(),
                 smp.new_p.data_ptr(), smp.idx.data_ptr(), gptr, dptr)
        return smp
    call("apn_sa_sample_seq", B, N, npoint, float(radius), nsample, p.data_ptr(), None,
         smp.fidx.data_ptr(), smp.new_p.data_ptr(), smp.idx.data_ptr(), gptr, dptr)
    return smp


@torch.no_grad()
def sample_and_query_many(ps, npoint, radius, nsample=K_NS, outs=None):
    ps = [p.contiguous() for p in ps]
    B, N, _ = ps[0].shape
    dev = ps[0].device
    if outs is None:
        outs = [Sampling(B, npoint, nsample, dev) for _ in ps]
    assert len(outs) == len(ps) and all(o.shape == (B, npoint, nsample) for o in outs)
    call = _Launcher(dev)
    for i in range(len(ps) + 1):
        a = i if i < len(ps) else None
        b = i - 1 if i >= 1 else None
        call("apn_sa_sample_overlap", B, N, npoint, float(radius), nsample,
             ps[a].data_ptr() if a is not None else None,
             outs[a].fidx.data_ptr() if a is not None else None,
             outs[a].new_p.data_ptr() if a is not None else None,
             ps[b].data_ptr() if b is not None else None,
             outs[b].new_p.data_ptr() if b is not None else None,
             outs[b].idx.data_ptr() if b is not None else None)
        if b is not None and outs[b].geo is not None:
            point_geo(ps[b], outs[b].new_p, outs[b].idx, radius, out=(outs[b].geo, outs[b].dd))
    return outs


class _SetAbstraction(torch.autograd.Function):
    @staticmethod
    def forward(ctx, p, f, w1, g1, b1, w2, g2, b2, ws, bs, mods):
        npoint, radius, conv1, bn1, conv2, bn2, skip_conv, relu, sync_bn, sampling = mods
        p = p.contiguous()
        f = f.contiguous()
        smp = sampling if sampling is not None else sample_and_query(p, npoint, radius, geo=True)
        fidx, new_p, idx = smp.fidx, smp.new_p, smp.idx
        if p.requires_grad:
            new_p = new_p.clone()
        fw = _Forward(p, f, new_p, idx, fidx, radius, conv1, bn1, conv2, bn2, skip_conv, relu,
                      sync_bn, tmap=smp.tmap, geo=smp.geo, dd=smp.dd, want_backward=any(ctx.needs_input_grad),
                      rowmap=smp.rowmap)
        ctx.fw = fw
        ctx.save_for_backward(p, f)
        ctx.set_materialize_grads(False)
        ctx.flags = (p.requires_grad, g1 is not None, b1 is not None, g2 is not None,
                     b2 is not None, ws is not None, bs is not None)
        ctx.mark_non_differentiable(new_p) if not p.requires_grad else None
        return new_p, fw.out

    @staticmethod
    def backward(ctx, g_newp_in, g_out):
        need_p, a1, a2, a3, a4, a5, a6 = ctx.flags
        fw = ctx.fw
        ctx.saved_tensors
        g = _backward(fw, g_out, need_p, need_p)
        g_p = g["p"]
        if need_p:
            gq = g["new_p"] if g_newp_in is None else g["new_p"] + g_newp_in
            g_p = g_p.scatter_add(1, fw.saved["fidx"].long().unsqueeze(-1).expand(-1, -1, 3), gq)
        ctx.fw = None
        return (g_p, g["f"], g["w1"], g["g1"] if a1 else None, g["b1"] if a2 else None, g["w2"],
                g["g2"] if a3 else None, g["b2"] if a4 else None, g["ws"] if a5 else None,
                g["bs"] if a6 else None, None)


def fused_set_abstraction(p, f, npoint, radius, conv1, bn1, conv2, bn2, skip_conv=None, relu=True,
                          sync_bn=False, sampling=None):
    assert skip_conv is None or isinstance(skip_conv, nn.Conv1d)
    ws = skip_conv.weight if skip_conv is not None else None
    bs = skip_conv.bias if skip_conv is not None else None
    return _SetAbstraction.apply(p, f, conv1.weight, bn1.weight, bn1.bias, conv2.weight, bn2.weight,
                                 bn2.bias, ws, bs,
                                 (npoint, radius, conv1, bn1, conv2, bn2, skip_conv, relu, sync_bn,
                                  sampling))
```

### include/adaptpoint_amd.h

```cpp
#ifndef ADAPTPOINT_AMD_H
#define ADAPTPOINT_AMD_H

#include <stddef.h>

#ifdef __cplusplus
extern "C" {
#endif

#define APN_OK 0
#define APN_EINVAL (-1)

#if defined(__GNUC__)
#define APN_API __attribute__((visibility("default")))
#else
#define APN_API
#endif

APN_API int apn_version(void);

APN_API const char *apn_error_string(int code);

APN_API const char *apn_build_flags(void);

APN_API int apn_furthest_point_sampling(int b, int n, int m, const float *xyz, float *temp,
                                int *idxs, void *stream);

APN_API int apn_ball_query(int b, int n, int m, float radius, int nsample, const float *new_xyz,
                   const float *xyz, int *idx, void *stream);

APN_API int apn_group_points(int b, int c, int n, int npoints, int nsample, const float *points,
                     const int *idx, float *out, void *stream);

APN_API int apn_group_points_grad(int b, int c, int n, int npoints, int nsample,
                          const float *grad_out, const int *idx, float *grad_points,
                          void *stream);

APN_API int apn_gather_points(int b, int c, int n, int npoints, const float *points,
                      const int *idx, float *out, void *stream);

APN_API int apn_gather_points_grad(int b, int c, int n, int npoints, const float *grad_out,
                           const int *idx, float *grad_points, void *stream);

APN_API int apn_resample_points(int b, int n, int c, int p_all, int s_cnt, int cx,
                                const float *points, const int *fidx, const int *choice,
                                float *pos, float *x, void *stream);

APN_API int apn_three_nn(int b, int n, int m, const float *unknown, const float *known,
                 float *dist2, int *idx, void *stream);

APN_API int apn_three_interpolate(int b, int c, int m, int n, const float *points, const int *idx,
                          const float *weight, float *out, void *stream);

APN_API int apn_three_interpolate_grad(int b, int c, int n, int m, const float *grad_out,
                               const int *idx, const float *weight, float *grad_points,
                               void *stream);


APN_API int apn_furthest_point_sampling_xyz(int b, int n, int m, const float *xyz, float *temp,
                                            int *idxs, float *new_xyz, void *stream);

APN_API int apn_ball_query_zero(int b, int n, int m, float radius, int nsample,
                                const float *new_xyz, const float *xyz, int *idx, void *stream);

APN_API int apn_sa_grid_blocks(int b, int m);
APN_API int apn_sa_grid_rows(int b, int m, int with_tile_map);
APN_API int apn_sa_bwd_main_rows(int b, int m);
APN_API int apn_sa_acc_words(int ncol);
APN_API int apn_zero_fill(void *base, long long bytes, void *stream);
APN_API int apn_debug_stamp(void *stamps, int slot, void *stream);
APN_API int apn_debug_vgpr_hold(int blocks, int turns, unsigned long long *bad, void *stream);
APN_API int apn_debug_vpk_probe(int blocks, int turns, int form, unsigned long long *bad, void *stream);


APN_API int apn_sa_geo_dd_doubles(int n);
APN_API int apn_sa_point_geo(int b, int n, int m, int nsample, float radius, const float *xyz,
                             const float *new_xyz, const int *idx, void *geo, void *dd, void *stream);

APN_API int apn_sa_prep_rows(int b, int n);
APN_API int apn_sa_prep_stats(int b, int n, const float *f, const void *geo, const void *dd, const float *w1,
                              int precision, int stats, void *ft, float *part1, void *zero, long long zero_words,
                              void *stream);

APN_API int apn_sa_reduce_rows(const float *part, int rows, int ncol, double count, double *out,
                               void *stream);
APN_API int apn_sa_reduce_acc(const void *acc, int ncol, double count, double *out, void *stream);

APN_API int apn_sa_bn_fold(const float *part, int rows, const double *sums, int c, double count,
                           const float *gamma, const float *beta, float eps, float momentum,
                           float *running_mean, float *running_var, void *num_batches_tracked,
                           int training, float *pack, const float *sgn_gamma, int sgn_c,
                           float *sgn_out, void *stream);

APN_API int apn_sa_fwd_main(int b, int n, int m, int precision, float radius, const float *xyz,
                            const float *new_xyz, const void *ft, const int *idx, const int *tmap, const float *w1,
                            const float *w2, const float *g1, const float *b1, float *rm1, float *rv1, void *nbt1,
                            float eps1, float mom1, int train1, double count, const float *part1, int rows1,
                            const double *sums1, float *pack1, const float *gamma2, float *ysel, void *ksel,
                            void *acc2, void *stream);

APN_API int apn_sa_fwd_out(int b, int n, int m, const float *ysel, const void *acc2, const double *sums2,
                           const float *g2, const float *b2, float *rm2, float *rv2, void *nbt2, float eps2,
                           float mom2, int train2, double count, float *pack2, const void *ft, int precision,
                           const int *fidx, const float *ws, const float *bs, int relu, float *out,
                           float *zero_base, long long zero_floats, void *stream);

APN_API int apn_sa_bwd_prep_rows(int b, int m);
APN_API int apn_sa_bwd_prep(int b, int n, int m, const float *g_out, long long gs_b,
                            long long gs_c, long long gs_m, const float *out, int relu,
                            const float *ysel, const float *pack2, const void *ft, int precision,
                            const int *fidx, const float *ws, float *goa, void *accS,
                            float *partWs, float *gip, const int *dup, void *stream);

APN_API int apn_sa_bwd_main(int b, int n, int m, int precision, float radius, const float *xyz,
                            const float *new_xyz, const void *ft, const int *idx, const int *tmap, const float *w1,
                            const float *w2, const float *pack1, const float *pack2, const void *accS,
                            const double *sumsS, double count, int train2, const float *goa, const void *ksel,
                            void *accT, float *partW2, const int *rowdst, float *GU, float *HA, float *HB,
                            void *stream);

APN_API int apn_sa_bwd_weight_rows(int b, int n);
APN_API int apn_sa_bwd_point_grads(int b, int n, int m, const float *GU, const int *pcnt_poff, const void *geo,
                                   const float *HA, const float *HB, const void *accT, const double *sumsT,
                                   double count, int train1, const float *pack1, const void *ft, int precision,
                                   const float *xyz, const float *new_xyz, const float *w1,
                                   const float *gip, float radius, float *partW, float *g_f,
                                   float *g_p, float *g_newp, void *stream);

APN_API int apn_sa_bwd_finalize(const float *partW, int rows_w, float radius, float *g_w1,
                                const float *partWs, int rows_s, float *g_ws, const float *partW2, int rows_2,
                                float *g_w2, const void *accS, const double *sumsS,
                                const void *accT, const double *sumsT, float *g_bs, float *g_g2, float *g_b2,
                                float *g_g1, float *g_b1, void *stream);

APN_API int apn_sa_debug_stamps(void *buf);

APN_API int apn_sa_forward_seq(
    int phases, int precision, int b, int n, int m, float radius, const float *xyz, const float *new_xyz,
    const float *f, const int *idx, const int *tmap, const int *fidx, const void *geo, const void *dd,
    const float *w1, const float *w2, const float *ws, const float *bs,
    const float *g1, const float *b1, float *rm1, float *rv1, void *nbt1, float eps1, float mom1,
    int train1,
    const float *g2, const float *b2, float *rm2, float *rv2, void *nbt2, float eps2, float mom2,
    int train2,
    double count, int relu, void *ft, float *part1, const double *sums1, const double *sums2,
    float *pack1, float *pack2, void *acc2, float *ysel, void *ksel,
    float *out, float *zero_base, long long zero_floats, void *stream);
APN_API int apn_sa_backward_seq(
    int phases, int precision, int b, int n, int m, float radius, const float *xyz, const float *new_xyz,
    const int *idx, const int *tmap, const int *fidx, const void *geo, const float *w1, const float *w2,
    const float *ws, const void *ft, const float *pack1, const float *pack2, const float *ysel,
    const void *ksel, const float *out, int relu, int train1, int train2, double count,
    const float *g_out, long long gs_b, long long gs_c, long long gs_m,
    void *zero_base, long long zero_bytes, float *gip, void *accS, void *accT,
    const int *pcnt_poff, const int *rowdst, float *GU,
    float *goa, float *partWs, float *partW2, float *partW, const double *sumsS, const double *sumsT,
    float *HA, float *HB,
    float *g_f, float *g_p, float *g_newp, float *g_w1, float *g_w2, float *g_g1, float *g_b1, float *g_g2,
    float *g_b2, float *g_ws, float *g_bs, void *stream);
APN_API int apn_sa_sample_overlap(int b, int n, int m, float radius, int nsample,
                                  const float *xyz_a, int *fidx_a, float *new_xyz_a,
                                  const float *xyz_b, const float *new_xyz_b, int *idx_b,
                                  void *stream);
APN_API int apn_furthest_point_sampling_nested(int b, int n, int m, const float *xyz, const int *tie_prev, int *idxs,
                                               float *new_xyz, int *tie_out, void *stream);
APN_API int apn_sa_sample_seq_nested(int b, int n, int m, float radius, int nsample, const float *xyz,
                                     const int *tie_prev, int *tie_out, int *fidx, float *new_xyz, int *idx, void *geo,
                                     void *dd, void *stream);
APN_API int apn_sa_sample_seq(int b, int n, int m, float radius, int nsample, const float *xyz,
                              float *temp, int *fidx, float *new_xyz, int *idx, void *geo, void *dd,
                              void *stream);

APN_API int apn_pointset_group_rows(int b, int m, int c);
APN_API int apn_pointset_group_max(int b, int n, int m, int c, int k, const float *points,
                                   const int *idx, const int *fidx, const float *alpha,
                                   const float *beta, float *out, void *ksel, void *stream);
APN_API int apn_pointset_group_max_grad(int b, int n, int m, int c, int k, const float *points,
                                        const int *idx, const int *fidx, const float *alpha,
                                        const void *ksel, const float *g_out, float *g_points,
                                        float *part, void *stream);

APN_API int apn_attention_small_max(void);
APN_API int apn_attention_small_fwd(int b, int m, int heads, const float *q, const float *k, const float *v,
                                    float *out, void *stream);
APN_API int apn_attention_small_bwd(int b, int m, int heads, const float *q, const float *k, const float *v,
                                    const float *g_out, float *dq, float *dk, float *dv, void *stream);
APN_API int apn_attention_prep(int b, int m, int heads, const float *q, const float *k,
                               const float *v, void *images, int for_backward, void *stream);
APN_API int apn_attention_fwd(int b, int m, int heads, const void *images, float *out, float *lse,
                              void *stream);
APN_API int apn_attention_bwd(int b, int m, int heads, const void *images, const float *out,
                              const float *lse, const float *g_out, void *scratch, float *dq,
                              float *dk, float *dv, void *stream);

APN_API int apn_sa_wide_grid(int b, int m);
APN_API int apn_sa_wide_tilemap_ints(int b, int m);
APN_API int apn_sa_wide_tilemap(int b, int m, int mode, const int *idx, int *tmap, void *stream);
APN_API int apn_sa_wide_tilemap_many(int count, int b, int m, int mode, const int *idx, int *tmap, void *stream);
APN_API int apn_sa_rowmap_places(int b, int n, int m);
APN_API int apn_sa_rowmap_ints(int b, int n);
APN_API int apn_sa_rowmap_many(int count, int b, int n, int m, const int *tmap, const int *fidx, int *pcnt_poff, int *rowdst, int *scratch,
                               void *stream);
APN_API int apn_sa_wide_colsum_chunks(int rows, int ncol);
APN_API int apn_sa_wide_colsum(const float *part, int rows, int ncol, double *scratch, double *out,
                               void *stream);
APN_API int apn_sa_wide_stats1(int b, int n, int m, int c_mid, const float *U, const float *V,
                               const int *idx, const int *tmap, float *part, void *stream);
APN_API int apn_sa_wide_fwd_main(int b, int n, int m, int c_mid, int c_out, const float *U, const float *V,
                                 const int *idx, const int *tmap, const void *w2_image, const float *pack1,
                                 const float *sgn2, float *ysel, void *ksel, float *part, void *stream);
APN_API int apn_sa_wide_bwd_main(int b, int n, int m, int c_mid, int c_out, const float *U, const float *V,
                                 const int *idx, const int *tmap, const void *z_image, const float *pack1,
                                 const float *evec, const float *goa, const void *ksel, float *GU,
                                 float *HA, float *HB, float *part, float *r_part, void *stream);
APN_API int apn_sa_wide_wgrad_fused(int c_mid);
APN_API int apn_sa_wide_image(const float *src0, int k0, int trans0, const float *src1, int kd, int nc, int ct,
                              void *image, void *stream);
APN_API int apn_sa_wide_bwd_prep_rows(int b, int m);
APN_API int apn_sa_wide_bwd_prep(int b, int m, int c_out, const float *g, long long gs_b, long long gs_c,
                                 long long gs_m, const float *ysel, const float *pack2, const float *out_act,
                                 float *gpre, float *goa, float *part_s, void *stream);
APN_API int apn_sa_wide_consts2(const float *part_s, int rows, const double *sums, int c_out,
                                const float *pack2, double count, int training, float *d2e2,
                                float *g_gamma2, float *g_beta2, void *stream);
APN_API int apn_sa_wide_consts1(const float *part_t, int rows, const double *sums, int c_mid,
                                const float *pack1, double count, int training, float *cabc,
                                float *g_gamma1, float *g_beta1, void *stream);
APN_API int apn_sa_wide_point_terms(int b, int n, int m, int c_mid, const float *cabc, const float *pack1,
                                    const float *U, const float *geo, const float *w1, int ldw, float radius,
                                    const float *GU, const int *pcnt_poff, const int *plist, float *G, float *HA,
                                    const float *HB, void *stream);
APN_API int apn_sa_wide_wgrad_splits(int b, int m, int c_mid);
APN_API int apn_sa_wide_wgrad(int b, int n, int m, int c_mid, int c_out, const float *U, const float *V,
                              const int *idx, const int *tmap, const float *pack1, const float *goa,
                              const void *ksel, int splits, float *r_part, void *stream);

APN_API int apn_sa_wide_csr(int b, int n, int m, const int *idx, const float *new_xyz, const int *tmap,
                            int *pcnt_poff, int *plist, float *geo, const int *fidx, int *fq, void *stream);
APN_API int apn_sa_wide_fwd_prep(int b, int c_in, int n, int m, int c_mid, int c_out, float radius, const float *f,
                                 const float *p, const float *new_p, const float *w1, const float *w2, float *U,
                                 float *V, void *w2_image, const int *fq, float *fs, const float *geo, float *part1,
                                 void *stream);
APN_API int apn_sa_wide_fwd_prep_rows(int b, int n, int m);
APN_API int apn_sa_wide_out(int b, int m, int c_out, const float *ysel, const float *pack2, int c_in,
                            const float *fs, const float *ws, const float *bs, int relu, float *out, void *stream);
APN_API int apn_sa_wide_bwd_mid(const float *part_s, int rows, const double *sums, int c_mid, int c_out,
                                const float *pack2, double count, int training, const float *w2, float *d2e2,
                                float *g_gamma2, float *g_beta2, float *evec, void *z_image, void *stream);
APN_API int apn_sa_wide_bwd_fin(const float *part_t, int rows, const double *sums, int c_mid, int c_out,
                                const float *pack1, double count, int training, float *cabc, float *g_gamma1,
                                float *g_beta1, const double *R, const float *d2e2, const float *w2, float *g_w2,
                                void *stream);
APN_API int apn_sa_wide_point_grads_rows(int b, int n);
APN_API int apn_sa_wide_point_grads(int b, int c_in, int n, int m, int c_mid, float radius, const float *GU,
                                    const int *pcnt_poff, const int *plist, const float *geo, const float *U,
                                    const float *f, const float *p, const float *new_p, const float *HA,
                                    const float *HB, const float *cabc, const float *pack1, const float *w1,
                                    int c_skip, const float *gpre, const int *fq, const float *fs, const float *ws,
                                    float *g_f, float *g_p, float *g_q, float *w_part, void *stream);
APN_API int apn_sa_wide_point_grads_cols(int c_in, int c_mid, int c_skip);
APN_API int apn_sa_wide_colsum_f32(const float *part, int rows, int ncol, float *out, void *stream);

APN_API int apn_pw_conv_tiles(int b, int n);
APN_API int apn_pw_conv_forward(int b, int c_in, int c_out, int n, int precision, const float *x, const float *w,
                                float *y, float *part, void *stream);
APN_API int apn_pw_bn_act(int b, int c, int n, const float *y, const float *part, int tiles, const float *gamma,
                          const float *beta, float eps, float momentum, int training, int relu, float *run_mean,
                          float *run_var, long long *batches, float *stat, float *out, void *stream);
APN_API int apn_pw_bn_act_grad_splits(int b, int c);
APN_API int apn_pw_bn_act_grad(int b, int c, int n, const float *g, const float *y, const float *stat, int training,
                               int relu, float *part_b, float *gy, float *g_gamma, float *g_beta, void *stream);
APN_API int apn_pw_conv_grad_input(int b, int c_in, int c_out, int n, int precision, const float *gy, const float *w,
                                   float *gx, void *stream);
APN_API int apn_pw_conv_grad_weight_splits(int b, int c_in, int c_out, int n);
APN_API int apn_pw_conv_grad_weight(int b, int c_in, int c_out, int n, int precision, const float *gy, const float *x,
                                    float *scratch, float *gw, void *stream);

APN_API int apn_pw_contract_splits(int nbatch, int r, int q, int k);
APN_API int apn_pw_contract(int nbatch, int r, int q, int k, const float *a, long long a_batch, int lda, int a_kcont,
                            const float *b, long long b_batch, int ldb, int b_kcont, float *d, long long d_batch, int ldd,
                            int splits, float *scratch, int precision, void *stream);
APN_API int apn_pw_contract2_splits(int which, int nbatch0, int r0, int q0, int k0, int nbatch1, int r1, int q1, int k1);
APN_API int apn_pw_contract2(int a_kcont, int b_kcont, int precision, const int *nbatch, const int *r, const int *q,
                             const int *k, const float *const *a, const long long *a_batch, const int *lda,
                             const float *const *b, const long long *b_batch, const int *ldb, float *const *d,
                             const long long *d_batch, const int *ldd, const int *splits, float *const *scratch,
                             void *stream);

APN_API int apn_fp_blend_stats(int b, int o, int m, int n, const float *a, const float *u, const int *idx,
                               const float *weight, float *y, float *part, int training, const float *gamma,
                               const float *beta, const float *run_mean, const float *run_var, float eps, int relu,
                               float *stat, float *out, void *stream);

APN_API int apn_pw_transpose(int nbatch, int r, int c, const float *in, float *out, void *stream);
APN_API int apn_three_nn_weights(long long n, const float *dist2, float *weight, void *stream);

APN_API int apn_anchor_transforms(int n, const float *prob, const float *keep, const float *axes, float r_range,
                                  float s_range, float t_range, float *lin, float *off, void *stream);
APN_API int apn_anchor_transforms_grad(int n, const float *prob, const float *keep, const float *axes, float r_range,
                                       float s_range, float t_range, const float *g_lin, const float *g_off,
                                       float *g_prob, void *stream);

APN_API int apn_deform_forward(int b, int n, int m, const float *xyz, const float *anchors, const float *lin,
                               const float *off, const float *axes, const float *mask, float sigma, float *z, float *stat,
                               float *out, void *stream);
APN_API int apn_deform_backward(int b, int n, int m, const float *xyz, const float *anchors, const float *axes,
                                const float *mask, float sigma, const float *z, const float *stat, const float *g_out,
                                float *g_lin, float *g_off, float *g_mask, void *stream);

APN_API int apn_pointwolf_params(int b, int m, const float *draws, int uniform, float r_range, float s_range,
                                 float t_range, float *lin, float *off, float *kaxes, void *stream);

APN_API int apn_rsmix_select(int b, int n, int c, const float *points, const int *draws, double r2, int knn_k,
                             int nsample, int *members, int *counts, void *stream);
APN_API int apn_rsmix_mix(int b, int n, int c, int nsample, const float *points, const int *draws, const int *members,
                          const int *counts, const int *pick, float *out, float *lam, void *stream);

#define APN_CT_PERMUTE 1
#define APN_CT_SCALE 2
#define APN_CT_HEIGHTS_SCALED 4
#define APN_CT_CENTER 8
#define APN_CT_NORMALIZE 16
#define APN_CT_ROTATE 32
#define APN_CT_UNIFORM 64
#define APN_CT_ANISOTROPIC 128
#define APN_CT_MIRROR 256
APN_API int apn_cloud_transform(int b, int n, int n_raw, int s, const float *raw, const int *rows, int flags,
                                int gravity_dim, const double *cfg, const int *perm, const float *params,
                                const float *uniforms, int *perm_out, float *params_out, float *out, void *stream);

APN_API int apn_cls_confusion(int b, int k, const float *logits, int ld, const int *target, const int *valid,
                              unsigned long long *cm, int *pred, void *stream);

APN_API int apn_pw_conv_max_tiles(int n);
APN_API int apn_pw_conv_max_forward(int b, int c_in, int c_out, int n, int precision, const float *x, const float *w,
                                    const float *bias, int relu, float *tile_val, int *tile_idx, float *out, int *idx,
                                    void *stream);
APN_API int apn_pw_conv_max_backward(int b, int c_in, int c_out, int n, const float *g_out, const float *out,
                                     const int *idx, const float *x, const float *w, int relu, float *xsel, float *g_x,
                                     float *g_w, float *g_bias, void *stream);

APN_API int apn_spectral_norm_blocks(int rows, int cols);
APN_API int apn_spectral_norm(int rows, int cols, const float *w, int training, float eps, float *u, float *v,
                              float *scratch, float *u_used, float *v_used, float *sigma, float *w_normalized,
                              void *stream);
APN_API int apn_spectral_norm_grad(int rows, int cols, const float *g, const float *w_normalized, const float *sigma,
                                   const float *u_used, const float *v_used, double *part, float *g_w, void *stream);

APN_API int apn_spectral_norm_many(int n_layers, const int *rows, const int *cols, const float *const *w, int training,
                                   float eps, float *const *u, float *const *v, float *const *scratch,
                                   float *const *u_used, float *const *v_used, float *const *sigma,
                                   float *const *w_normalized, void *stream);
APN_API int apn_spectral_norm_grad_many(int n_layers, const int *rows, const int *cols, const float *const *g,
                                        const float *const *w_normalized, const float *const *sigma,
                                        const float *const *u_used, const float *const *v_used, double *const *part,
                                        float *const *g_w, void *stream);

APN_API int apn_la_pool_rows(int b, int n);
APN_API int apn_la_pool_fwd(int b, int n, int c, int nsample, float radius, const float *U, const float *xyz,
                            const float *wp, int ldw, const int *idx, const float *gamma, float *ext, void *sel,
                            float *ysum, double *part, void *stream);
APN_API int apn_la_stats_fold(const double *part, int rows, int c, double count, double *sums, void *stream);
APN_API int apn_la_pool_bwd(int b, int n, int c, int nsample, float radius, const float *gsel, const void *sel,
                            const int *tmap, const int *pcnt_poff, const int *plist, const float *geo, const float *U,
                            const float *xyz, const float *ysum, const float *de, const float *wp, int ldw, float *dU,
                            float *dT, float *dp, void *stream);

APN_API int apn_knn_query(int b, int n, int m, int c, int k, const float *support, const float *query, int *idx,
                          float *dist2, void *stream);

APN_API int apn_knn_dilated(int b, int n, int m, int c, int kd, int k, int dilation, const int *slots,
                            const float *support, const float *query, int *idx, float *dist2, void *stream);

APN_API int apn_ec_pool_rows(int b, int n);
APN_API int apn_ec_pool_fwd(int b, int n, int c, int k, const float *uv, int ld, const int *idx, const float *gamma,
                            float *ext, void *sel, float *ysum, double *part, void *stream);
APN_API int apn_ec_out(int b, int n, int c, const float *ext, const float *pack, float slope, float *out, void *stream);
APN_API int apn_ec_bwd_prep_rows(int b, int n);
APN_API int apn_ec_bwd_prep(int b, int n, int c, const float *g, long long gs_b, long long gs_c, long long gs_n,
                            const float *ext, const float *pack, float slope, float *gsel, float *part_s, void *stream);
APN_API int apn_ec_out_res(int b, int n, int c, const float *ext, const float *pack, float slope, const float *res,
                           long long rs_b, long long rs_c, long long rs_n, float *out, void *stream);
APN_API int apn_ec_bwd_prep_act(int b, int n, int c, const float *g, long long gs_b, long long gs_c, long long gs_n,
                                const float *ext, const float *pack, float slope, float *gsel, float *part_s,
                                void *stream);
APN_API int apn_ec_csr(int b, int n, int k, const int *idx, int *pcnt_poff, int *plist, int *scratch, void *stream);
APN_API int apn_ec_pool_bwd(int b, int n, int c, int k, const float *gsel, const void *sel, const int *pcnt_poff,
                            const int *plist, const float *uv, int ld, const float *ysum, const float *de, float *duv,
                            void *stream);

APN_API int apn_chamfer_max_points(void);
APN_API int apn_chamfer_forward(int b, int n, int m, const float *xyz1, const float *xyz2, float *dist1, float *dist2,
                                int *idx1, int *idx2, void *stream);
APN_API int apn_chamfer_backward(int b, int n, int m, const float *xyz1, const float *xyz2, const int *idx1,
                                 const int *idx2, const float *grad_dist1, const float *grad_dist2, float *grad_xyz1,
                                 float *grad_xyz2, void *stream);

APN_API int apn_emd_max_points(void);
APN_API int apn_emd_one_launch_max(void);
APN_API int apn_emd_cost_parts(int n);
APN_API int apn_emd_ratios(int b, int n, int m, const float *xyz1, const float *xyz2, float *ratio_l, float *ratio_r,
                           float *state, void *stream);
APN_API int apn_emd_match(int b, int n, int m, const float *xyz1, const float *xyz2, const float *ratio_l,
                          const float *ratio_r, float *match, void *stream);
APN_API int apn_emd_cost(int b, int n, int m, const float *xyz1, const float *xyz2, const float *match,
                         const float *ratio_l, const float *ratio_r, float *part, float *cost, void *stream);
APN_API int apn_emd_cost_grad(int b, int n, int m, const float *grad_cost, const float *xyz1, const float *xyz2,
                              const float *match, const float *ratio_l, const float *ratio_r, float *grad1, float *grad2,
                              void *stream);

APN_API int apn_po_knn_query(int b, int n, int m, int k, const float *xyz, const float *new_xyz, const int *offset,
                             const int *new_offset, int *idx, float *dist2, void *stream);
APN_API int apn_po_ball_query(int b, int n, int m, float radius, int nsample, const float *xyz, const float *new_xyz,
                              const int *offset, const int *new_offset, int *idx, void *stream);
APN_API int apn_po_furthest_sampling(int b, int n_max, const float *xyz, const int *offset, const int *new_offset,
                                     float *tmp, int *idx, void *stream);
APN_API int apn_po_csr(int n, int m, int k, const int *idx, int *pcnt_poff, int *plist, int *scratch, void *stream);
APN_API int apn_po_grouping_fwd(int n, int m, int k, int c, const float *input, const int *idx, float *out, void *stream);
APN_API int apn_po_grouping_bwd(int n, int m, int k, int c, const float *grad_out, const int *pcnt_poff, const int *plist,
                                float *grad_input, void *stream);
APN_API int apn_po_interpolation_fwd(int n, int m, int k, int c, const float *input, const int *idx, const float *weight,
                                     float *out, void *stream);
APN_API int apn_po_interpolation_bwd(int n, int m, int k, int c, const float *grad_out, const float *weight,
                                     const int *pcnt_poff, const int *plist, float *grad_input, void *stream);
APN_API int apn_po_subtraction_fwd(int n, int m, int k, int c, const float *input1, const float *input2, const int *idx,
                                   float *out, void *stream);
APN_API int apn_po_subtraction_bwd(int n, int m, int k, int c, const float *grad_out, const int *pcnt_poff,
                                   const int *plist, float *grad_input1, float *grad_input2, void *stream);
APN_API int apn_po_aggregation_fwd(int n, int m, int k, int c, int w_c, const float *input, const float *position,
                                   const float *weight, const int *idx, float *out, void *stream);
APN_API int apn_po_aggregation_bwd(int n, int m, int k, int c, int w_c, const float *input, const float *position,
                                   const float *weight, const int *idx, const float *grad_out, const int *pcnt_poff,
                                   const int *plist, float *grad_input, float *grad_position, float *grad_weight,
                                   void *stream);

APN_API int apn_pt_rows(int n, int k, int c);
APN_API int apn_pt_mid_rows(int n, int k, int c);
APN_API int apn_pt_rel_stats(int n, int k, int c, const float *qkv, int ld, const float *h, const int *idx,
                             const float *wts, double *part, void *stream);
APN_API int apn_pt_fold(const double *part, int rows, int width, double *sums, void *stream);
APN_API int apn_pt_colsum_rows(int n);
APN_API int apn_pt_colsum(int n, int width, const float *src, int ld, double *part, void *stream);
APN_API int apn_pt_mid(int n, int k, int c, const float *qkv, int ld, const float *h, const int *idx, const float *wts,
                       const float *bn, float *t, double *part, void *stream);
APN_API int apn_pt_attend(int n, int k, int c, const float *qkv, int ld, const float *h, const int *idx,
                          const float *wts, const float *bn, const float *t, float *a, float *out, void *stream);
APN_API int apn_pt_attend_bwd(int n, int k, int c, const float *qkv, int ld, const float *h, const int *idx,
                              const float *wts, const float *bn, const float *t, const float *a, const float *go,
                              float *g1, double *part, void *stream);
APN_API int apn_pt_mid_bwd(int n, int k, int c, const float *qkv, int ld, const float *h, const int *idx,
                           const float *wts, const float *bn, const float *de, const float *t, const float *g1,
                           double *part, void *stream);
APN_API int apn_pt_rel_bwd(int n, int k, int c, const float *qkv, int ld, const float *h, const int *idx,
                           const float *wts, const float *bn, const float *de, const float *t, const float *g1,
                           const float *a, const float *go, float *dr, float *dh, float *dqkv, int ldg, double *part,
                           void *stream);
APN_API int apn_pt_scatter_bwd(int n, int k, int c, const float *dr, const float *go, const float *a,
                               const int *pcnt_poff, const int *plist, float *dqkv, int ldg, void *stream);

APN_API int apn_vg_scratch_ints(int n);
APN_API int apn_vg_voxelize(int b, int n, int is_double, const void *coord, double vx, double vy, double vz,
                            const int *offset, int *scratch, int *voxel_of, int *count, int *start, int *idx_sort,
                            int *new_offset, int *stats, void *stream);
APN_API int apn_vg_mean_fwd(int n, int m, int c, const float *values, const int *idx_sort, const int *start,
                            const int *count, float *out, void *stream);
APN_API int apn_vg_mean_bwd(int n, int m, int c, const float *grad_out, const int *voxel_of, const int *count,
                            float *grad_values, void *stream);

APN_API int apn_rl_moment_rows(int b, int n, int k);
APN_API int apn_rl_bwd_rows(int b, int n, int k, int c);
APN_API int apn_rl_moments(int b, int n, int k, const float *coords, const int *idx, const float *dist, int sqrt_dist,
                           double *part, double *mom, void *stream);
APN_API int apn_rl_fold(int c, const double *mom, double count, const float *w, const float *bias, const float *gamma,
                        const float *beta, float eps, float momentum, int training, float *running_mean,
                        float *running_var, long long *num_batches_tracked, float *wf, double *stat, void *stream);
APN_API int apn_rl_forward(int b, int n, int k, int c, const float *coords, const int *idx, const float *dist,
                           int sqrt_dist, const float *wf, const float *at, float *pooled, void *stream);
APN_API int apn_rl_backward(int b, int n, int k, int c, const float *coords, const int *idx, const float *dist,
                            int sqrt_dist, const float *wf, const float *a, const float *at, const float *dpooled,
                            float *part, void *stream);
APN_API int apn_rl_finalize(int c, int rows, const float *part, const double *mom, double count, const float *w,
                            const float *bias, const float *gamma, const double *stat, int training, double *sums,
                            float *grads, void *stream);

APN_API int apn_ag_moment_rows(int s);
APN_API int apn_ag_point_rows(int n);
APN_API int apn_ag_moments(int b, int n, int s, int k, int c, const float *x, const int *idx, const int *fps_idx,
                           double *part, void *stream);
APN_API int apn_ag_fold(int rows, int ncol, const double *part, double *out, void *stream);
APN_API int apn_ag_combine_fwd(int b, int n, int s, int k, int o, const float *pq, const int *idx, const int *fps_idx,
                               const float *r, const float *c0, float *y, float *part, int training, const float *gamma,
                               const float *beta, const float *run_mean, const float *run_var, float eps, int relu,
                               float *stat, float *out, void *stream);
APN_API int apn_ag_combine_bwd(int b, int n, int s, int k, int o, const float *gyt, const float *r, const float *pq,
                               const int *pcnt_poff_i, const int *plist_i, const int *pcnt_poff_a, const int *plist_a,
                               float *dpq, double *part_dr, double *part_c0, void *stream);
APN_API int apn_ag_sigma_bwd(int b, int n, int s, int k, int c, const float *x, const int *idx, const int *fps_idx,
                             const float *kappa, const float *mu, const int *pcnt_poff_i, const int *plist_i,
                             const int *pcnt_poff_a, const int *plist_a, float *dx, void *stream);
APN_API int apn_ag_res_relu_max(int b, int o, int s, int k, const float *z, const float *h, float *out, void *sel,
                                void *stream);
APN_API int apn_ag_res_relu_max_grad(int b, int o, int s, int k, const float *g, const float *out, const void *sel,
                                     float *gz, float *gh, void *stream);

APN_API int apn_furthest_point_sampling_tuned(int b, int n, int m, const float *xyz, float *temp,
                                              int *idx, int waves, int algo, void *stream);

APN_API int apn_fps_debug_stamps(int b, int n, int m, const float *xyz, float *temp, int *idxs,
                                 unsigned long long *dbg, void *stream);

#ifdef __cplusplus
}
#endif
#endif
```

Before: 122,400.

## Move skip-branch gradient GEMMs from bwd_prep into point-grads kernel via inverse linked lists

The skip-connection gradient work (g_f contribution through ws and the ws weight gradient) moves out of bwd_prep and into bwd_point_grads. bwd_prep now only writes the raw upstream gradient gq and builds a per-point inverse map (pinv plus a next-chain via atomicExch) from sampled points back to query rows. The point-grads kernel walks that chain, sums the gradients, and adds the skip MFMA into its existing accumulator. It also computes the partWs tiles per point block. This drops the gip zero-fill, the atomicAdd scatter and the extra gip read. The cost is pointer-chasing for duplicated picks and more shared memory in the point-grads kernel.

```diff
diff --git a/adaptpoint_amd/_lib.py b/adaptpoint_amd/_lib.py
--- a/adaptpoint_amd/_lib.py
+++ b/adaptpoint_amd/_lib.py
@@ -53,11 +53,11 @@
                       + [_c_int] + [_c_void_p] * 3 + [_c_int] + [_c_void_p] * 2 + [_c_longlong, _c_void_p],
     "apn_sa_bwd_prep_rows": [_c_int] * 2,
     "apn_sa_bwd_prep": [_c_int] * 3 + [_c_void_p] + [_c_longlong] * 3 + [_c_void_p] + [_c_int]
-                       + [_c_void_p] * 3 + [_c_int] + [_c_void_p] * 8,
+                       + [_c_void_p] * 10,
     "apn_sa_bwd_main": [_c_int] * 4 + [_c_float] + [_c_void_p] * 11 + [_c_double, _c_int] + [_c_void_p] * 9,
     "apn_sa_bwd_weight_rows": [_c_int] * 2,
     "apn_sa_bwd_point_grads": [_c_int] * 3 + [_c_void_p] * 7 + [_c_double, _c_int] + [_c_void_p] * 2 + [_c_int]
-                              + [_c_void_p] * 4 + [_c_float] + [_c_void_p] * 5,
+                              + [_c_void_p] * 8 + [_c_float] + [_c_void_p] * 5,
     "apn_sa_bwd_finalize": [_c_void_p, _c_int, _c_float, _c_void_p, _c_void_p, _c_int, _c_void_p, _c_void_p, _c_int]
                            + [_c_void_p] * 11,
     "apn_sa_forward_seq": ([_c_int] * 5 + [_c_float] + [_c_void_p] * 12
@@ -67,7 +67,7 @@
     "apn_sa_backward_seq": ([_c_int] * 5 + [_c_float] + [_c_void_p] * 15 + [_c_int] * 3
                             + [_c_double] + [_c_void_p] + [_c_longlong] * 3 + [_c_void_p]
                             + [_c_longlong]
-                            + [_c_void_p] * 26),
+                            + [_c_void_p] * 28),
     "apn_attention_small_max": [],
     "apn_attention_small_fwd": [_c_int] * 3 + [_c_void_p] * 5,
     "apn_attention_small_bwd": [_c_int] * 3 + [_c_void_p] * 8,
diff --git a/adaptpoint_amd/csrc/sa_glue.hip b/adaptpoint_amd/csrc/sa_glue.hip
--- a/adaptpoint_amd/csrc/sa_glue.hip
+++ b/adaptpoint_amd/csrc/sa_glue.hip
@@ -307,37 +307,30 @@
                                                            const float *__restrict__ out, int relu,
                                                            const float *__restrict__ ysel,
                                                            const float *__restrict__ pack2,
-                                                           const __bf16 *__restrict__ ft,
-                                                           const __bf16 *__restrict__ ft_lo,
                                                            const int *__restrict__ fidx,
-                                                           const float *__restrict__ ws,
                                                            float *__restrict__ goa,
                                                            unsigned long long *__restrict__ accS,
-                                                           float *__restrict__ partWs,
-                                                           float *__restrict__ gip,
+                                                           float *__restrict__ gq,
+                                                           int *__restrict__ pinv,
+                                                           int *__restrict__ next,
                                                            const int *__restrict__ dup) {
     constexpr int NT = QT * 16, NW = NT / 64, HALVES = 64 / QT;
     __shared__ float tile[QT][65];
     __shared__ float red[NW][2][64];
-    __shared__ __attribute__((aligned(16))) float sfi[QT][36];
-    __shared__ float sws[64][33];
-    __shared__ int ssrc[QT];
-    constexpr int DW = QT == 32 ? 4 : 2;
-    __shared__ float sdfi[DW][QT][33];
     const int cloud = blockIdx.y, m0 = blockIdx.x * QT;
     const int tx = threadIdx.x & 63, ty = threadIdx.x >> 6;
     const int ql = tx % QT, hh = tx / QT;
     critical_stream_priority();
     wg_stamp(0);
-    const bool distinct = dup && dup[cloud] == 0;
     const int qc = m0 + ql < m ? m0 + ql : m - 1;
     const float *outp = relu ? out : g_out;
+    const long long os_b = relu ? 64ll * m : gs_b, os_c = relu ? (long long)m : gs_c, os_m = relu ? 1ll : gs_m;
     float gv[4], ov[4];
 #pragma unroll
     for (int k = 0; k < 4; ++k) {
         const int c = (ty + NW * k) * HALVES + hh;
         gv[k] = g_out[cloud * gs_b + c * gs_c + qc * gs_m];
-        ov[k] = relu ? outp[((size_t)cloud * 64 + c) * m + qc] : 1.0f;
+        ov[k] = outp[cloud * os_b + c * os_c + qc * os_m];
     }
     float ys[4];
 #pragma unroll
@@ -345,13 +338,26 @@
         const int q = m0 + ty + NW * k;
         ys[k] = ysel[((size_t)cloud * m + (q < m ? q : m - 1)) * 64 + tx];
     }
-    if (ws) stage_skip_operands<NT, QT, 33, 36>(cloud, n, m, m0, ft, ft_lo, fidx, ws, sws, sfi, ssrc);
+    const int pick = fidx ? fidx[(size_t)cloud * m + qc] : -1;
+    const bool distinct = dup && dup[cloud] == 0;
 #pragma unroll
     for (int k = 0; k < 4; ++k) {
         const int c = (ty + NW * k) * HALVES + hh;
-        tile[ql][c] = (m0 + ql < m && ov[k] > 0.0f) ? gv[k] : 0.0f;
+        tile[ql][c] = (m0 + ql < m && (!relu || ov[k] > 0.0f)) ? gv[k] : 0.0f;
     }
     const float sc = pack2[tx], mu = pack2[128 + tx], iv = pack2[192 + tx];
+    asm volatile("" :: "v"(pick), "s"((int)distinct));
+    if (fidx && threadIdx.x < QT && m0 + ql < m) {
+        const int q = m0 + ql;
+        const bool valid = (unsigned)pick < (unsigned)n;
+        int *slot = pinv + (size_t)cloud * n + (valid ? pick : 0);
+        if (distinct) {
+            if (valid) *slot = q + 1;
+            next[(size_t)cloud * m + q] = 0;
+        } else {
+            next[(size_t)cloud * m + q] = valid ? atomicExch(slot, q + 1) : 0;
+        }
+    }
     wg_stamp(1);
     __syncthreads();
     wg_stamp(2);
@@ -363,6 +369,7 @@
             const float g = tile[j][tx];
             const float gs = g * sc;
             goa[((size_t)cloud * m + q) * 64 + tx] = gs;
+            if (gq) gq[((size_t)cloud * m + q) * 64 + tx] = g;
             s1 += g;
             s2 += g * ((ys[k] - mu) * iv);
         }
@@ -379,59 +386,8 @@
         for (int k = 0; k < NW; ++k) sacc += red[k][ty][tx];
     }
     wg_stamp(5);
-    if (ws) {
-        constexpr int QB = QT / 32;
-        const int r = tx & 31, h = tx >> 5;
-        if (ty < DW * QB) {
-            const int qb = ty / DW, part = ty % DW;
-            f32x16 acc = {0};
-#pragma unroll
-            for (int s4 = 0; s4 < 4 / DW; ++s4) {
-                const int st = (4 / DW) * part + s4;
-                float av[8], bv[8];
-#pragma unroll
-                for (int j = 0; j < 8; ++j) {
-                    av[j] = tile[32 * qb + r][16 * st + 8 * h + j];
-                    bv[j] = sws[16 * st + 8 * h + j][r];
-                }
-                acc = mfma<2>(make_frag<2>(av), make_frag<2>(bv), acc);
-            }
-#pragma unroll
-            for (int e = 0; e < 16; ++e)
-                sdfi[part][32 * qb + acc_row(e, h)][r] = acc[e];
-        } else if (ty < DW * QB + 2) {
-            const int cb = ty - DW * QB;
-            f32x16 acc = {0};
-#pragma unroll
-            for (int st = 0; st < QT / 16; ++st) {
-                float av[8], bv[8];
-#pragma unroll
-                for (int j = 0; j < 8; ++j) {
-                    av[j] = tile[16 * st + 8 * h + j][32 * cb + r];
-                    bv[j] = sfi[16 * st + 8 * h + j][r];
-                }
-                acc = mfma<2>(make_frag<2>(av), make_frag<2>(bv), acc);
-            }
-#pragma unroll
-            for (int e = 0; e < 16; ++e)
-                partWs[blk * 2048 + (32 * cb + acc_row(e, h)) * 32 + r] = acc[e];
-        }
-        __syncthreads();
-#pragma unroll
-        for (int k = 0; k < QT * 32 / NT; ++k) {
-            const int o = threadIdx.x + NT * k, q = o >> 5, i = o & 31;
-            float v = sdfi[0][q][i] + sdfi[1][q][i];
-            if (DW == 4) v += sdfi[DW - 2][q][i] + sdfi[DW - 1][q][i];
-            float *dst = gip + ((size_t)cloud * n + ssrc[q]) * 32 + i;
-            if (m0 + q < m) {
-                if (distinct) *dst = v;
-                else atomicAdd(dst, v);
-            }
-        }
-        wg_stamp(6);
-    }
     if (ty < 2) acc_add(accS, 128, (int)(blk % ACC_COPIES), ty * 64 + tx, sacc);
-    wg_stamp(7);
+    wg_stamp(6);
 }
 
 constexpr int WG_PTS = 64;
@@ -445,14 +401,17 @@
     const double *__restrict__ sumsT, double count, int train1,
     const float *__restrict__ pack1, const __bf16 *__restrict__ ft,
     const __bf16 *__restrict__ ft_lo, const float *__restrict__ xyz,
-    const float *__restrict__ new_xyz, const float *__restrict__ w1, const float *__restrict__ gip,
+    const float *__restrict__ new_xyz, const float *__restrict__ w1, int m, const float *__restrict__ ws,
+    const float *__restrict__ gq, const int *__restrict__ pinv, const int *__restrict__ next,
+    float *__restrict__ partWs,
     float inv_r, float *__restrict__ partW, float *__restrict__ g_f, float *__restrict__ g_p,
     float *__restrict__ g_q) {
     __shared__ __attribute__((aligned(16))) float swt[35][36];
     __shared__ __attribute__((aligned(16))) float swr[32][36];
     __shared__ float sG[WG_PTS][33];
     __shared__ float sH[WG_PTS][33];
-    __shared__ float sI[WG_PTS][33];
+    __shared__ float sGs[WG_PTS][65];
+    __shared__ __attribute__((aligned(16))) float sWs[64][36];
     __shared__ float sB[WG_PTS][41];
     __shared__ float sGeo[WG_PTS][4];
     __shared__ float sc[5][32];
@@ -465,18 +424,23 @@
     const int q0 = block * WG_PTS;
     const int n_here = n - n0 < WG_PTS ? n - n0 : WG_PTS;
     const int c_ld = tid & 31;
-    float f_hi[PG_K], f_lo[PG_K], g_i[PG_K], h_a[PG_K], h_b[PG_K];
+    float f_hi[PG_K], f_lo[PG_K], h_a[PG_K], h_b[PG_K];
     const int g_pt = tid >> 3, g_c4 = (tid & 7) * 4;
-    int r_cnt, r_off;
+    int r_cnt, r_off, r_pick;
     {
         const size_t gp = p0 + (g_pt < n_here ? g_pt : 0);
         r_cnt = g_pt < n_here ? pcnt[gp] : 0;
         r_off = poff[gp];
+        r_pick = (ws ? pinv : pcnt)[gp];
     }
     float4 a_g = make_float4(0.f, 0.f, 0.f, 0.f);
+    float ws_v[4] = {0.f, 0.f, 0.f, 0.f};
+    if (ws) {
+#pragma unroll
+        for (int k = 0; k < 4; ++k) ws_v[k] = ws[tid + PG_NT * k];
+    }
     {
         const __bf16 *lo_tab = ft_lo ? ft_lo : ft;
-        const float *gip_tab = gip ? gip : HA;
 #pragma unroll
         for (int k = 0; k < PG_K; ++k) {
             const int pt = (tid >> 5) + (PG_NT / 32) * k;
@@ -484,7 +448,6 @@
             const size_t qr = (size_t)(q0 + pt < total_q ? q0 + pt : 0) * 32 + c_ld;
             f_hi[k] = (float)ft[pr];
             f_lo[k] = (float)lo_tab[pr];
-            g_i[k] = gip_tab[gip ? pr : qr];
             h_a[k] = HA[qr];
             h_b[k] = HB[qr];
         }
@@ -520,18 +483,54 @@
         sc[tid < 32 ? 2 : 1][c] = val;
         if (tid < 32) sc[0][c] = sca;
     } else if (tid >= 96 && tid < 160) sc[3 + ((tid - 96) >> 5)][tid & 31] = pack1[64 + tid - 96];
-    {
-        const float *rows = GU + (size_t)(r_cnt > 0 ? r_off : 0) * 32 + g_c4;
-        for (int j0 = 0; j0 < r_cnt; j0 += PG_RB) {
-            float4 v[PG_RB];
-#pragma unroll
-            for (int u = 0; u < PG_RB; ++u) {
-                const int j = j0 + u < r_cnt ? j0 + u : r_cnt - 1;
-                v[u] = *reinterpret_cast<const float4 *>(rows + (size_t)j * 32);
-            }
-#pragma unroll
-            for (int u = 0; u < PG_RB; ++u)
-                if (j0 + u < r_cnt) { a_g.x += v[u].x; a_g.y += v[u].y; a_g.z += v[u].z; a_g.w += v[u].w; }
+    const float *rows = GU + (size_t)(r_cnt > 0 ? r_off : 0) * 32 + g_c4;
+    float4 v_first[PG_RB];
+#pragma unroll
+    for (int u = 0; u < PG_RB; ++u) {
+        const int j = u < r_cnt ? u : (r_cnt > 0 ? r_cnt - 1 : 0);
+        v_first[u] = *reinterpret_cast<const float4 *>(rows + (size_t)j * 32);
+    }
+    const float *gq_c = nullptr;
+    const int *next_c = nullptr;
+    bool picked = false;
+    int nx = 0;
+    float4 s_lo = make_float4(0.f, 0.f, 0.f, 0.f), s_hi = s_lo;
+    if (ws) {
+        gq_c = gq + (size_t)cloud * m * 64 + g_c4;
+        next_c = next + (size_t)cloud * m;
+        picked = g_pt < n_here && (unsigned)(r_pick - 1) < (unsigned)m;
+        const int qf = picked ? r_pick - 1 : 0;
+        s_lo = *reinterpret_cast<const float4 *>(gq_c + (size_t)qf * 64);
+        s_hi = *reinterpret_cast<const float4 *>(gq_c + (size_t)qf * 64 + 32);
+        nx = next_c[qf];
+    }
+#pragma unroll
+    for (int u = 0; u < PG_RB; ++u)
+        if (u < r_cnt) { a_g.x += v_first[u].x; a_g.y += v_first[u].y; a_g.z += v_first[u].z; a_g.w += v_first[u].w; }
+    for (int j0 = PG_RB; j0 < r_cnt; j0 += PG_RB) {
+        float4 v[PG_RB];
+#pragma unroll
+        for (int u = 0; u < PG_RB; ++u) {
+            const int j = j0 + u < r_cnt ? j0 + u : r_cnt - 1;
+            v[u] = *reinterpret_cast<const float4 *>(rows + (size_t)j * 32);
+        }
+#pragma unroll
+        for (int u = 0; u < PG_RB; ++u)
+            if (j0 + u < r_cnt) { a_g.x += v[u].x; a_g.y += v[u].y; a_g.z += v[u].z; a_g.w += v[u].w; }
+    }
+    if (ws) {
+        if (!picked) {
+            s_lo = make_float4(0.f, 0.f, 0.f, 0.f);
+            s_hi = s_lo;
+            nx = 0;
+        }
+        for (int hops = 1; (unsigned)(nx - 1) < (unsigned)m && hops < m; ++hops) {
+            const size_t q = (size_t)(nx - 1);
+            const float4 v0 = *reinterpret_cast<const float4 *>(gq_c + q * 64);
+            const float4 v1 = *reinterpret_cast<const float4 *>(gq_c + q * 64 + 32);
+            nx = next_c[q];
+            s_lo.x += v0.x; s_lo.y += v0.y; s_lo.z += v0.z; s_lo.w += v0.w;
+            s_hi.x += v1.x; s_hi.y += v1.y; s_hi.z += v1.z; s_hi.w += v1.w;
         }
     }
     wg_stamp(1);
@@ -545,12 +544,18 @@
             const int pt = (tid >> 5) + (PG_NT / 32) * k;
             const bool ok = pt < n_here;
             sB[pt][6 + c] = ok ? f_hi[k] + (ft_lo ? f_lo[k] : 0.0f) : 0.0f;
-            sI[pt][c] = (gip && ok) ? g_i[k] : 0.0f;
             sH[pt][c] = q0 + pt < total_q ? __builtin_fmaf(ca, h_a[k], __builtin_fmaf(cb, h_b[k], cc * 32.0f)) : 0.0f;
         }
     }
     sG[g_pt][g_c4] = a_g.x; sG[g_pt][g_c4 + 1] = a_g.y;
     sG[g_pt][g_c4 + 2] = a_g.z; sG[g_pt][g_c4 + 3] = a_g.w;
+    if (ws) {
+        float *gs_row = &sGs[g_pt][g_c4];
+        gs_row[0] = s_lo.x; gs_row[1] = s_lo.y; gs_row[2] = s_lo.z; gs_row[3] = s_lo.w;
+        gs_row[32] = s_hi.x; gs_row[33] = s_hi.y; gs_row[34] = s_hi.z; gs_row[35] = s_hi.w;
+#pragma unroll
+        for (int k = 0; k < 4; ++k) sWs[(tid >> 5) + (PG_NT / 32) * k][tid & 31] = ws_v[k];
+    }
     if (tid < WG_PTS * 3) {
         const int pt = tid / 3, d = tid % 3;
         const float xv = xq_v[0], qv = xq_v[1];
@@ -630,12 +635,40 @@
                 for (int j = 0; j < 8; ++j) bv[j] = sG[32 * pb + r][16 * st + 8 * h + j];
                 acc = mfma<2>(make_frag<2>(av), make_frag<2>(bv), acc);
             }
+            if (ws) {
+#pragma unroll
+                for (int st = 0; st < 4; ++st) {
+                    float av[8], bv[8];
+#pragma unroll
+                    for (int j = 0; j < 8; ++j) {
+                        av[j] = sWs[16 * st + 8 * h + j][r];
+                        bv[j] = sGs[32 * pb + r][16 * st + 8 * h + j];
+                    }
+                    acc = mfma<2>(make_frag<2>(av), make_frag<2>(bv), acc);
+                }
+            }
             const int pt = 32 * pb + r;
 #pragma unroll
             for (int e = 0; e < 16; ++e) {
                 const int i = acc_row(e, h);
-                if (pt < n_here) g_f[((size_t)cloud * 32 + i) * n + n0 + pt] = acc[e] + sI[pt][i];
+                if (pt < n_here) g_f[((size_t)cloud * 32 + i) * n + n0 + pt] = acc[e];
             }
+        } else if (ty < 7 && ws) {
+            const int cb = ty - 5;
+            f32x16 acc = {0};
+#pragma unroll
+            for (int st = 0; st < WG_PTS / 16; ++st) {
+                float av[8], bv[8];
+#pragma unroll
+                for (int j = 0; j < 8; ++j) {
+                    av[j] = sGs[16 * st + 8 * h + j][32 * cb + r];
+                    bv[j] = sB[16 * st + 8 * h + j][6 + r];
+                }
+                acc = mfma<2>(make_frag<2>(av), make_frag<2>(bv), acc);
+            }
+            float *row = partWs + (size_t)block * 2048;
+#pragma unroll
+            for (int e = 0; e < 16; ++e) row[(32 * cb + acc_row(e, h)) * 32 + r] = acc[e];
         }
     }
     if (!g_p && !g_q) {
@@ -831,23 +864,20 @@
 
 extern "C" int apn_sa_bwd_prep(int b, int n, int m, const float *g_out, long long gs_b,
                                long long gs_c, long long gs_m, const float *out, int relu,
-                               const float *ysel, const float *pack2, const void *ft, int precision,
-                               const int *fidx, const float *ws, float *goa, void *accS,
-                               float *partWs, float *gip, const int *dup, void *stream) {
+                               const float *ysel, const float *pack2, const int *fidx, float *goa, void *accS,
+                               float *gq, int *pinv, int *next, const int *dup, void *stream) {
     if (b <= 0 || m <= 0 || b > 65535 || !g_out || !ysel || !pack2 || !goa || !accS) return APN_EINVAL;
     if (relu && !out) return APN_EINVAL;
-    if (ws && (!ft || !fidx || !partWs || !gip || n <= 0 || (precision != 1 && precision != 2)))
-        return APN_EINVAL;
-    const __bf16 *hi = (const __bf16 *)ft;
-    const __bf16 *lo = (ws && precision == 2) ? hi + (size_t)b * n * 32 : nullptr;
+    if (fidx && (!gq || !pinv || !next || n <= 0)) return APN_EINVAL;
+    if (!fidx) gq = nullptr;
     if (apn_sa_glue_tile(b, m) == 32)
         hipLaunchKernelGGL(apn::bwd_prep_kernel<32>, dim3((m + 31) / 32, b), dim3(512), 0, APN_ST, n, m, g_out,
-                           gs_b, gs_c, gs_m, out, relu, ysel, pack2, hi, lo, fidx, ws, goa, (unsigned long long *)accS,
-                           partWs, gip, dup);
+                           gs_b, gs_c, gs_m, out, relu, ysel, pack2, fidx, goa, (unsigned long long *)accS, gq, pinv,
+                           next, dup);
     else
         hipLaunchKernelGGL(apn::bwd_prep_kernel<64>, dim3((m + 63) / 64, b), dim3(1024), 0, APN_ST, n, m, g_out,
-                           gs_b, gs_c, gs_m, out, relu, ysel, pack2, hi, lo, fidx, ws, goa, (unsigned long long *)accS,
-                           partWs, gip, dup);
+                           gs_b, gs_c, gs_m, out, relu, ysel, pack2, fidx, goa, (unsigned long long *)accS, gq, pinv,
+                           next, dup);
     APN_LAUNCH_CHECK();
     return APN_OK;
 }
@@ -864,9 +894,11 @@
                                       const float *HA, const float *HB, const void *accT, const double *sumsT,
                                       double count, int train1, const float *pack1, const void *ft, int precision,
                                       const float *xyz, const float *new_xyz, const float *w1,
-                                      const float *gip, float radius, float *partW, float *g_f,
+                                      const float *ws, const float *gq, const int *pinv, const int *next,
+                                      float *partWs, float radius, float *partW, float *g_f,
                                       float *g_p, float *g_newp, void *stream) {
     if (b <= 0 || n <= 0 || m <= 0 || b > 65535) return APN_EINVAL;
+    if (ws && (!gq || !pinv || !next || !partWs || ((uintptr_t)gq & 15))) return APN_EINVAL;
     if (!GU || !pcnt_poff || !geo || !HA || !HB || (!accT && !sumsT) || !pack1 || !ft || !xyz || !new_xyz || !w1 || !partW ||
         !g_f)
         return APN_EINVAL;
@@ -878,7 +910,8 @@
                        dim3(apn::PG_NT), 0, APN_ST, n, b * m, precision == 2 ? 1 : 0, GU, pcnt_poff,
                        pcnt_poff + (size_t)b * n, (const long long *)geo, HA, HB,
                        (const unsigned long long *)accT, sumsT, count, train1,
-                       pack1, hi, lo, xyz, new_xyz, w1, gip, 1.0f / radius, partW, g_f, g_p, g_newp);
+                       pack1, hi, lo, xyz, new_xyz, w1, m, ws, gq, pinv, next, partWs, 1.0f / radius, partW, g_f, g_p,
+                       g_newp);
     APN_LAUNCH_CHECK();
     return APN_OK;
 }
diff --git a/adaptpoint_amd/csrc/sa_seq.hip b/adaptpoint_amd/csrc/sa_seq.hip
--- a/adaptpoint_amd/csrc/sa_seq.hip
+++ b/adaptpoint_amd/csrc/sa_seq.hip
@@ -59,7 +59,7 @@
     const float *ws, const void *ft, const float *pack1, const float *pack2, const float *ysel,
     const void *ksel, const float *out, int relu, int train1, int train2, double count,
     const float *g_out, long long gs_b, long long gs_c, long long gs_m,
-    void *zero_base, long long zero_bytes, float *gip, void *accS, void *accT,
+    void *zero_base, long long zero_bytes, float *gq, int *pinv, int *next, void *accS, void *accT,
     const int *pcnt_poff, const int *rowdst, float *GU,
     float *goa, float *partWs, float *partW2, float *partW, const double *sumsS, const double *sumsT,
     float *HA, float *HB,
@@ -67,8 +67,8 @@
     float *g_b2, float *g_ws, float *g_bs, void *stream) {
     if (phases & 1) {
         if (zero_bytes) APN_TRY(apn_zero_fill(zero_base, zero_bytes, stream));
-        APN_TRY(apn_sa_bwd_prep(b, n, m, g_out, gs_b, gs_c, gs_m, out, relu, ysel, pack2, ws ? ft : nullptr, precision,
-                                ws ? fidx : nullptr, ws, goa, accS, partWs, gip,
+        APN_TRY(apn_sa_bwd_prep(b, n, m, g_out, gs_b, gs_c, gs_m, out, relu, ysel, pack2, ws ? fidx : nullptr, goa, accS,
+                                ws ? gq : nullptr, pinv, next,
                                 pcnt_poff ? pcnt_poff + 2ll * b * n : nullptr, stream));
     }
     if (phases & 2)
@@ -76,9 +76,9 @@
                                 sumsS, count, train2, goa, ksel, accT, partW2, rowdst, GU, HA, HB, stream));
     if (phases & 4) {
         APN_TRY(apn_sa_bwd_point_grads(b, n, m, GU, pcnt_poff, geo, HA, HB, accT, sumsT, count, train1, pack1, ft, precision, xyz,
-                                       new_xyz, w1, gip, radius, partW, g_f, g_p, g_newp, stream));
+                                       new_xyz, w1, ws, gq, pinv, next, partWs, radius, partW, g_f, g_p, g_newp, stream));
         APN_TRY(apn_sa_bwd_finalize(partW, apn_sa_bwd_weight_rows(b, n), radius, g_w1, partWs,
-                                    apn_sa_bwd_prep_rows(b, m), g_ws, partW2, apn_sa_bwd_main_rows(b, m), g_w2, accS,
+                                    apn_sa_bwd_weight_rows(b, n), g_ws, partW2, apn_sa_bwd_main_rows(b, m), g_w2, accS,
                                     sumsS, accT, sumsT, g_bs, g_g2, g_b2, g_g1, g_b1, stream));
     }
     return APN_OK;
diff --git a/adaptpoint_amd/fused.py b/adaptpoint_amd/fused.py
--- a/adaptpoint_amd/fused.py
+++ b/adaptpoint_amd/fused.py
@@ -163,7 +163,7 @@
                                ("ysel", B * M * C_OUT), ("ksel", B * M * C_OUT // 4),
                                ("part1", rows1 * 64), ("acc2", _acc_floats(128))])
         out = torch.empty(B, C_OUT, M, dtype=torch.float32, device=dev)
-        self.zsizes = (([("gip", B * N * C_MID)] if ws is not None else [])
+        self.zsizes = (([("pinv", B * N)] if ws is not None else [])
                        + [("accS", _acc_floats(128)), ("accT", _acc_floats(64))])
         self.zviews = self.zbuf = None
         if want_backward:
@@ -218,7 +218,6 @@
     lib = _lib.load()
     call = _Launcher(dev)
     rows = lib.apn_sa_bwd_main_rows(B, M)
-    prow = lib.apn_sa_bwd_prep_rows(B, M)
     wrows = lib.apn_sa_bwd_weight_rows(B, N)
 
     prezeroed = fw.zbuf is not None
@@ -226,7 +225,8 @@
     if sv["rowmap"] is None:
         raise RuntimeError("fused set abstraction: backward without a row map (the forward was run with want_backward=False)")
     pcnt_poff, rowdst = sv["rowmap"]
-    sizes = zsizes + [("goa", B * M * C_OUT), ("partWs", prow * C_OUT * C_IN if has_skip else 0),
+    sizes = zsizes + [("goa", B * M * C_OUT), ("gq", B * M * C_OUT if has_skip else 0), ("next", B * M if has_skip else 0),
+                      ("partWs", wrows * C_OUT * C_IN if has_skip else 0),
                       ("partW2", rows * C_OUT * C_MID), ("partW", wrows * 32 * 38),
                       ("HA", B * M * C_MID), ("HB", B * M * C_MID), ("GU", lib.apn_sa_rowmap_places(B, N, M) * C_MID)]
     v, buf = _carve(dev, sizes)
@@ -247,14 +247,15 @@
     def run(phases, sumsS=None, sumsT=None):
         if PER_KERNEL_LAUNCH:
             return _backward_per_kernel(call, phases, fw, sv, g_out, buf, zero_floats, v, g, sumsS,
-                                        sumsT, g_f, g_p, g_newp, rows, prow, wrows, has_skip, pcnt_poff, rowdst)
+                                        sumsT, g_f, g_p, g_newp, rows, wrows, has_skip, pcnt_poff, rowdst)
         call("apn_sa_backward_seq", phases, fw.prec, B, N, M, fw.radius, sv["p"].data_ptr(),
              sv["new_p"].data_ptr(), sv["idx"].data_ptr(), _ptr(sv["tmap"]), _ptr(sv["fidx"]), sv["geo"].data_ptr(),
              w1.data_ptr(), w2.data_ptr(), _ptr(ws), sv["ft"].data_ptr(), sv["pack1"].data_ptr(),
              sv["pack2"].data_ptr(), sv["ysel"].data_ptr(), sv["ksel"].data_ptr(),
              fw.out.data_ptr(), fw.relu, 1 if fw.train1 else 0, 1 if fw.train2 else 0, float(P),
              g_out.data_ptr(), gs[0], gs[1], gs[2], buf.data_ptr(), zero_floats * 4,
-             v["gip"].data_ptr() if has_skip else None, v["accS"].data_ptr(),
+             v["gq"].data_ptr() if has_skip else None, v["pinv"].data_ptr() if has_skip else None,
+             v["next"].data_ptr() if has_skip else None, v["accS"].data_ptr(),
              v["accT"].data_ptr(), pcnt_poff.data_ptr(), rowdst.data_ptr(), v["GU"].data_ptr(), v["goa"].data_ptr(),
              v["partWs"].data_ptr() if has_skip else None, v["partW2"].data_ptr(), v["partW"].data_ptr(),
              _ptr(sumsS), _ptr(sumsT), v["HA"].data_ptr(), v["HB"].data_ptr(),
@@ -293,17 +294,16 @@
 
 
 def _backward_per_kernel(call, phases, fw, sv, g_out, buf, zero_floats, v, g, sumsS, sumsT, g_f, g_p,
-                         g_newp, rows, prow, wrows, has_skip, pcnt_poff, rowdst):
+                         g_newp, rows, wrows, has_skip, pcnt_poff, rowdst):
     B, N, M = fw.dims
     w1, w2, ws, P = sv["w1"], sv["w2"], sv["ws"], float(sv["count"])
-    gip = v["gip"].data_ptr() if has_skip else None
+    gq, pinv, nxt = ((v["gq"].data_ptr(), v["pinv"].data_ptr(), v["next"].data_ptr()) if has_skip else (None, None, None))
     if phases & 1:
         if zero_floats:
             call("apn_zero_fill", buf.data_ptr(), zero_floats * 4)
         call("apn_sa_bwd_prep", B, N, M, g_out.data_ptr(), *g_out.stride(), fw.out.data_ptr(), fw.relu,
-             sv["ysel"].data_ptr(), sv["pack2"].data_ptr(), sv["ft"].data_ptr() if has_skip else None,
-             fw.prec, _ptr(sv["fidx"]) if has_skip else None, _ptr(ws), v["goa"].data_ptr(),
-             v["accS"].data_ptr(), v["partWs"].data_ptr() if has_skip else None, gip,
+             sv["ysel"].data_ptr(), sv["pack2"].data_ptr(), _ptr(sv["fidx"]) if has_skip else None, v["goa"].data_ptr(),
+             v["accS"].data_ptr(), gq, pinv, nxt,
              pcnt_poff.data_ptr() + 8 * B * N)
     if phases & 2:
         call("apn_sa_bwd_main", B, N, M, fw.prec, fw.radius, sv["p"].data_ptr(), sv["new_p"].data_ptr(),
@@ -315,9 +315,10 @@
         call("apn_sa_bwd_point_grads", B, N, M, v["GU"].data_ptr(), pcnt_poff.data_ptr(), sv["geo"].data_ptr(),
              v["HA"].data_ptr(), v["HB"].data_ptr(), v["accT"].data_ptr(), _ptr(sumsT), P, 1 if fw.train1 else 0,
              sv["pack1"].data_ptr(), sv["ft"].data_ptr(), fw.prec, sv["p"].data_ptr(), sv["new_p"].data_ptr(),
-             w1.data_ptr(), gip, fw.radius, v["partW"].data_ptr(), g_f.data_ptr(), _ptr(g_p), _ptr(g_newp))
+             w1.data_ptr(), _ptr(ws), gq, pinv, nxt, v["partWs"].data_ptr() if has_skip else None, fw.radius,
+             v["partW"].data_ptr(), g_f.data_ptr(), _ptr(g_p), _ptr(g_newp))
         call("apn_sa_bwd_finalize", v["partW"].data_ptr(), wrows, fw.radius, g["w1"].data_ptr(),
-             v["partWs"].data_ptr() if has_skip else None, prow, g["ws"].data_ptr() if has_skip else None,
+             v["partWs"].data_ptr() if has_skip else None, wrows, g["ws"].data_ptr() if has_skip else None,
              v["partW2"].data_ptr(), rows, g["w2"].data_ptr(), v["accS"].data_ptr(), _ptr(sumsS),
              v["accT"].data_ptr(), _ptr(sumsT), g["bs"].data_ptr() if (has_skip and sv["has_bs"]) else None,
              g["g2"].data_ptr(), g["b2"].data_ptr(), g["g1"].data_ptr(), g["b1"].data_ptr())
diff --git a/include/adaptpoint_amd.h b/include/adaptpoint_amd.h
--- a/include/adaptpoint_amd.h
+++ b/include/adaptpoint_amd.h
@@ -107,9 +107,8 @@
 APN_API int apn_sa_bwd_prep_rows(int b, int m);
 APN_API int apn_sa_bwd_prep(int b, int n, int m, const float *g_out, long long gs_b,
                             long long gs_c, long long gs_m, const float *out, int relu,
-                            const float *ysel, const float *pack2, const void *ft, int precision,
-                            const int *fidx, const float *ws, float *goa, void *accS,
-                            float *partWs, float *gip, const int *dup, void *stream);
+                            const float *ysel, const float *pack2, const int *fidx, float *goa, void *accS,
+                            float *gq, int *pinv, int *next, const int *dup, void *stream);
 
 APN_API int apn_sa_bwd_main(int b, int n, int m, int precision, float radius, const float *xyz,
                             const float *new_xyz, const void *ft, const int *idx, const int *tmap, const float *w1,
@@ -123,7 +122,8 @@
                                    const float *HA, const float *HB, const void *accT, const double *sumsT,
                                    double count, int train1, const float *pack1, const void *ft, int precision,
                                    const float *xyz, const float *new_xyz, const float *w1,
-                                   const float *gip, float radius, float *partW, float *g_f,
+                                   const float *ws, const float *gq, const int *pinv, const int *next,
+                                   float *partWs, float radius, float *partW, float *g_f,
                                    float *g_p, float *g_newp, void *stream);
 
 APN_API int apn_sa_bwd_finalize(const float *partW, int rows_w, float radius, float *g_w1,
@@ -151,7 +151,7 @@
     const float *ws, const void *ft, const float *pack1, const float *pack2, const float *ysel,
     const void *ksel, const float *out, int relu, int train1, int train2, double count,
     const float *g_out, long long gs_b, long long gs_c, long long gs_m,
-    void *zero_base, long long zero_bytes, float *gip, void *accS, void *accT,
+    void *zero_base, long long zero_bytes, float *gq, int *pinv, int *next, void *accS, void *accT,
     const int *pcnt_poff, const int *rowdst, float *GU,
     float *goa, float *partWs, float *partW2, float *partW, const double *sumsS, const double *sumsT,
     float *HA, float *HB,
```

After: 122,100. About the same (-0.3%).
